# sapeirone/EgoPack

Measured on AMD Instinct MI355X. Metric: clip-seqs/sec training, AR+LTA+PNR multi-task, higher is better.
Workload: dtype bf16; 1 GPU; MTL pre-train AR+LTA+PNR (BASELINE config 3): per GPU B=64 seqs/task x T=32 nodes, 3x1536-d Omnivore-shaped features, H=1024, TRN hidden 1024 (dropout 0.5), depth 3, k=1, Adam; graph mode, fused backbone pass; global_batch=192, parallelism=dp1, trainable_params=25003272, capture=one graph, input=resident in HBM before the timed region, master_weights=f32, mode=bf16, activations=bf16

## Files before the change

__graft_entry__.py:

```python
from __future__ import annotations

import subprocess
import sys
from pathlib import Path

REPO = Path(__file__).resolve().parent
if str(REPO) not in sys.path:
    sys.path.insert(0, str(REPO))


def build() -> None:
    from egopack_amd import build as b
    lib = b.build_library(force=False, verbose=False)
    assert lib.exists()
    from egopack_amd import _lib
    handle = _lib.load()
    missing = [s for s in [*_lib.header_symbols(), *_lib.optim_header_symbols(), *_lib.optim_groups_header_symbols(),
                            *_lib.ema_header_symbols(), *_lib.ce_balanced_header_symbols(),
                            *_lib.bce_balanced_header_symbols()] if not hasattr(handle, s)]
    if missing:
        raise RuntimeError(f"libegopack_hip.so does not export: {missing}")
    import egopack_amd.engine
    import egopack_amd.models


def smoke() -> None:
    import torch
    if not torch.cuda.is_available():
        raise RuntimeError("smoke() needs a GPU")
    build()
    from egopack_amd import data as D
    from egopack_amd import engine, ops
    from egopack_amd.criterion import BCEWithLogitsNone, CrossEntropyNone, MetricSelectorWrapper
    from egopack_amd.models import Graph
    from egopack_amd.models.tasks import LTATask, OSCCTask, PNRTask, RecognitionTask
    from egopack_amd.optim import FlatAdam
    from oracle import path as O
    from oracle import pyg_ops as P

    torch.manual_seed(1)
    F_IN, S, H, HP, heads = 64, 3, 128, 96, (13, 17)
    trn = {"_target_": "egopack_amd.models.temporal_pooling.trn_pooling.TRNPooling", "dropout": 0.0, "hidden_size": HP}
    model = Graph(F_IN, hidden_size=H, depth=3, temporal_pooling=trn, num_segments=S)
    tasks = {"ar": RecognitionTask(H, H, heads), "oscc": OSCCTask(H, H), "lta": LTATask(H, H, heads), "pnr": PNRTask(H, H)}
    names = {"ar": "task/recognition", "oscc": "task/oscc", "lta": "task/lta", "pnr": "task/pnr"}
    sds = {"temporal_graph": {k: v.clone() for k, v in model.state_dict().items()}}
    for t, n in names.items():
        sds[n] = {k: v.clone() for k, v in tasks[t].state_dict().items()}
    host = {}
    for t, T in (("ar", 9), ("lta", 12), ("pnr", 8)):
        ds = D.SyntheticTaskDataset(t, 4, T, S, F_IN, heads, k=1, seed=3)
        host[t] = D.collate([ds[i] for i in range(4)])
    weights = {"ar": 1.0, "oscc": 0.0, "lta": 0.5, "pnr": 2.0}

    class DS:
        has_joint_label, num_labels = False, 2
    crit = {"ar": MetricSelectorWrapper(CrossEntropyNone(), DS()), "lta": MetricSelectorWrapper(CrossEntropyNone(), DS()),
            "oscc": CrossEntropyNone(), "pnr": BCEWithLogitsNone()}
    model.cuda()
    for t in tasks.values():
        t.cuda()
    params = [*model.parameters(), *(p for t in tasks.values() for p in t.parameters())]
    opt = FlatAdam(params, lr=1e-3, weight_decay=1e-5)
    step = engine.MTLStep(model, tasks, crit, weights, opt, fused_backbone=True)
    dev = {t: b.to("cuda") for t, b in host.items()}
    with ops.compute_mode("f32"):
        total, vectors = step.step(dev)
    torch.cuda.synchronize()

    leaf = {g: {k: (v.clone().requires_grad_(True) if v.is_floating_point() and not k.endswith("frequency") else v)
                for k, v in sd.items()} for g, sd in sds.items()}
    obatches = {t: P.OData(**{k: v for k, v in b.__dict__.items() if torch.is_tensor(v) or k == "num_graphs"})
# ... 19 lines not shown
```

egopack_amd/_lib.py:

```python
from __future__ import annotations

import ctypes as C
import os
import re
from pathlib import Path

import torch

HERE = Path(__file__).resolve().parent
LIB_PATH = Path(os.environ["EGK_LIB_PATH"]) if os.environ.get("EGK_LIB_PATH") else HERE / "libegopack_hip.so"
HEADER = HERE.parent / "include" / "egopack_hip.h"
OPTIM_HEADER = HERE.parent / "include" / "egopack_optim.h"
OPTIM_GROUPS_HEADER = HERE.parent / "include" / "egopack_optim_groups.h"

EMA_HEADER = HERE.parent / "include" / "egopack_ema.h"
CE_BALANCED_HEADER = HERE.parent / "include" / "egopack_ce_balanced.h"
BCE_BALANCED_HEADER = HERE.parent / "include" / "egopack_bce_balanced.h"

vp, i32, i64, u64, f32 = C.c_void_p, C.c_int32, C.c_int64, C.c_uint64, C.c_float


class GemmDesc(C.Structure):
    _fields_ = [
        ("M", i32), ("N", i32), ("K1", i32), ("K2", i32),
        ("A1", vp), ("A2", vp), ("B1", vp), ("B2", vp),
        ("lda1", i64), ("lda2", i64), ("ldb1", i64), ("ldb2", i64),
        ("transA", i32), ("transB", i32), ("a_dtype", i32), ("b_dtype", i32),
        ("compute", i32),
        ("C", vp), ("ldc", i64), ("c_dtype", i32),
        ("accumulate", i32), ("act", i32), ("alpha", f32),
        ("bias", vp), ("residual", vp), ("ldr", i64), ("r_dtype", i32),
        ("splitk", i32), ("ws", vp), ("ws_bytes", i64), ("dbias", vp),
        ("st_mode", i32), ("st_nseg", i32), ("st_min_seg_rows", i32), ("st_seg_ptr", vp), ("st_ws", vp), ("st_x", vp),
        ("st_ldx", i64), ("st_stats", vp), ("st_w", vp), ("st_b", vp), ("st_slope", f32),
        ("n_extra", i32), ("xK", i32 * 4), ("xA", vp * 4), ("xB", vp * 4), ("xlda", i64 * 4), ("xldb", i64 * 4),
        ("op_f16", i32),
    ]


class HostDataset(C.Structure):
    _fields_ = [("T", i32), ("S", i32), ("train", i32), ("y_heads", i32), ("L", i64), ("y_elems", i64), ("heavy_in_launch", i64),
                ("live_share", C.c_double),
                ("y", vp), ("pos", vp), ("tau", vp), ("first", vp), ("vlen", vp), ("starts", vp), ("ends", vp),
                ("n_tmpl", i64), ("e_max", i64), ("h_max", i64), ("th_max", i64),
                ("t_e", vp), ("t_ei", vp), ("t_col", vp), ("t_tcol", vp), ("t_tw", vp), ("t_rp", vp), ("t_trp", vp), ("t_band", vp),
                ("t_nh", vp), ("t_nth", vp), ("t_hv", vp), ("t_thv", vp), ("t_dmax", vp), ("t_tdmax", vp)]


class HostBatch(C.Structure):
    _fields_ = [("E", i64), ("heavy_cap", i64), ("t_heavy_cap", i64), ("live_cap", i64),
                ("y", vp), ("pos", vp), ("batch", vp), ("ptr", vp), ("ptr32", vp), ("x_idx", vp), ("edge_index", vp),
                ("rowptr", vp), ("col", vp), ("t_rowptr", vp), ("t_col", vp), ("t_wgt", vp), ("band", vp), ("heavy", vp), ("t_heavy", vp),
                ("live_idx", vp), ("live_inv", vp), ("live_y", vp),
                ("n_heavy", i64), ("n_t_heavy", i64), ("n_live", i64), ("pos_min", i64), ("pos_max", i64),
                ("heavy_mode", i32), ("t_heavy_mode", i32), ("edge_cap", i64), ("live_ap_first", i64), ("live_ap_step", i64)]


class HostPart(C.Structure):
    _fields_ = [("n_nodes", i64), ("E", i64), ("n_heavy", i64), ("n_t_heavy", i64), ("edge_stride", i64), ("pos_min", i64), ("pos_max", i64),
                ("pos", vp), ("edge_index", vp), ("rowptr", vp), ("col", vp), ("t_rowptr", vp), ("t_col", vp), ("t_wgt", vp), ("band", vp),
                ("heavy", vp), ("t_heavy", vp), ("heavy_mode", i32), ("t_heavy_mode", i32)]


class HostMerged(C.Structure):
    _fields_ = [("edge_cap", i64), ("pos", vp), ("edge_index", vp), ("rowptr", vp), ("col", vp), ("t_rowptr", vp), ("t_col", vp),
                ("t_wgt", vp), ("band", vp), ("heavy", vp), ("t_heavy", vp), ("seg_ptr", vp),
                ("n_nodes", i64), ("E", i64), ("min_seg_rows", i64), ("pos_min", i64), ("pos_max", i64),
                ("heavy_mode", i32), ("t_heavy_mode", i32)]


class CETask(C.Structure):
    _fields_ = [("logits", vp * 4), ("ld", i64 * 4), ("C", i32 * 4), ("pad", i32 * 4), ("dcol", i64 * 4), ("n_heads", i32),
                ("y", vp), ("y_stride", i64), ("loss", vp), ("dlogits", vp), ("ldd", i64), ("rows", i32), ("gscale", f32)]


class CEWTask(C.Structure):
    _fields_ = [("base", CETask), ("weight", vp * 4), ("offset", vp * 4)]


class OptimDesc(C.Structure):
    _fields_ = [("rule", i32), ("g_dtype", i32), ("n", i64), ("p", vp), ("g", vp), ("state0", vp), ("state1", vp), ("hyper", vp),
                ("t_dev", vp), ("beta1", C.c_double), ("beta2", C.c_double), ("eps", f32), ("weight_decay", f32), ("momentum", f32), ("dampening", f32),
                ("nesterov", i32), ("bf16_shadow", vp), ("bf16_lo_shadow", vp), ("bump_word", vp), ("bump", i64), ("gate", vp)]


class OptimGroups(C.Structure):
    _fields_ = [("base", i64), ("n_seg", i32), ("n_groups", i32), ("seg_begin", vp), ("seg_group", vp), ("group_hyper", vp)]


class EmaDesc(C.Structure):
    _fields_ = [("ema", vp), ("decay", C.c_double), ("warmup", i32)]


OPT_ADAM, OPT_ADAMW, OPT_SGD = 0, 1, 2

SIGNATURES = {
    "egk_version": (C.c_int, []),
    "egk_last_error": (C.c_char_p, []),
    "egk_prof_enable": (C.c_int, [C.c_int]),
    "egk_prof_reset": (C.c_int, []),
    "egk_prof_count": (C.c_int, []),
    "egk_prof_get": (C.c_int, [C.c_int, C.c_char_p, C.c_int, C.POINTER(i64), C.POINTER(C.c_double),
                               C.POINTER(C.c_double), C.POINTER(C.c_double)]),
    "egk_stamp": (C.c_int, [vp, vp, i32]),
    "egk_tee_split_next": (C.c_int, [vp, vp, i64]),
    "egk_gemm": (C.c_int, [vp, C.POINTER(GemmDesc)]),
    "egk_gemm_stats_blocks": (C.c_int, [C.POINTER(GemmDesc)]),
    "egk_gemm_grouped": (C.c_int, [vp, C.POINTER(GemmDesc), i32]),
    "egk_gemm_ws_bytes": (i64, [C.POINTER(GemmDesc)]),
    "egk_gemm_splitk": (C.c_int, [i32, i32, i32, i32]),
    "egk_gemm_set_pipeline": (C.c_int, [i32]),
    "egk_colsum_ws_len": (C.c_int, [i32, i32]),
    "egk_colsum": (C.c_int, [vp, vp, i64, i32, i32, vp, i32, vp, i32]),
    "egk_rowln_fwd": (C.c_int, [vp, vp, vp, vp, vp, vp, vp, vp, i32, i32, f32, i32, f32, u64, u64, vp, i32]),
    "egk_rowln_bwd_ws_rows": (C.c_int, [i32]),
    "egk_rowln_bwd": (C.c_int, [vp, vp, vp, vp, vp, vp, vp, vp, vp, vp, vp, vp, i32, i32, i32, f32, i32]),
    "egk_ln_bwd_reduce": (C.c_int, [vp, vp, vp, vp, i32, i32, i32]),
    "egk_ln_bwd_reduce_multi": (C.c_int, [vp, vp, vp, vp, vp, vp, vp, i32]),
    "egk_rowln_group_fwd": (C.c_int, [vp, vp, vp, vp, vp, i32, vp, vp, vp, i32, f32, i32, i32]),
    "egk_rowln_group_bwd": (C.c_int, [vp, vp, vp, vp, vp, vp, i32, vp, vp, vp, vp, i32, i32, i32]),
    "egk_graphln_ws_bytes": (i64, [i32, i32, i32]),
    "egk_graphln_fwd": (C.c_int, [vp, vp, vp, vp, vp, vp, vp, i32, i32, i32, f32, f32, vp, i32]),
    "egk_graphln_bwd": (C.c_int, [vp, vp, vp, vp, vp, vp, vp, vp, vp, vp, i32, i32, i32, f32, f32, vp, i32]),
    "egk_rowdot_ws_rows": (i32, [i32]),
    "egk_rowdot_bce": (C.c_int, [vp, vp, vp, vp, vp, vp, vp, vp, vp, i32, i32, f32, i32]),
    "egk_rowdot_reduce": (C.c_int, [vp, vp, vp, vp, i32, i32]),
    "egk_rowdot_ce2_max_rows": (i32, []),
    "egk_rowdot_ce2": (C.c_int, [vp, vp, vp, vp, vp, vp, vp, vp, vp, vp, vp, i32, i32, f32, f32, i32]),
    "egk_rowdot_ce2_multi": (C.c_int, [vp, i32, vp, vp, vp, vp, vp, vp, vp, vp, vp, vp, i32, i32, i32, f32, f32, i32]),
    "egk_graphln_stats_blocks": (i32, [i32]),
    "egk_graphln_stats": (C.c_int, [vp, vp, vp, i32, i32, i32, vp, i32]),
    "egk_graphln_bwd_stats": (C.c_int, [vp, vp, vp, vp, vp, vp, vp, i32, i32, i32, f32, vp, i32]),
    "egk_graphln_bwd_finish": (C.c_int, [vp, vp, vp, vp, vp, vp, vp, vp, vp, vp, i32, i32, i32, f32, f32, vp, i32, vp, i32]),
    "egk_graphln_fwd_apply": (C.c_int, [vp, vp, vp, vp, vp, vp, vp, i32, i32, i32, f32, f32, vp, i32, i32]),
    "egk_graphln_bwd_apply": (C.c_int, [vp, vp, vp, vp, vp, vp, vp, vp, i32, i32, i32, f32, f32, vp, i32, vp, i32]),
    "egk_pe_table": (C.c_int, [vp, vp, i64, i32, i32, vp]),
    "egk_pe_add_table": (C.c_int, [vp, vp, vp, vp, vp, i64, i32, vp, i32, i32, i32]),
    "egk_pe_add": (C.c_int, [vp, vp, vp, vp, vp, i32, i32, i32]),
    "egk_csr_gather": (C.c_int, [vp, vp, vp, vp, vp, vp, vp, i32, i32, i32, vp, i32, vp, i32]),
    "egk_csr_gather_banded": (C.c_int, [vp, vp, vp, vp, vp, vp, i32, i32, i32, vp, i32, vp, i32]),
    "egk_csr_heavy_ws_bytes": (i64, [i32, i32]),
    "egk_csr_heavy_threshold": (i32, []),
    "egk_gather_max_fwd": (C.c_int, [vp, vp, vp, vp, vp, vp, i32, i32, i32, i32]),
    "egk_gather_max_group_fwd": (C.c_int, [vp, vp, vp, vp, i32, vp, vp, i32, i32, i32, i32]),
    "egk_gather_max_tune": (C.c_int, [i32]),
# ... 42 lines not shown
    "egk_weighted_sums_acc": (C.c_int, [vp, vp, vp, vp, i32, vp, vp]),
    "egk_fill_scaled_multi": (C.c_int, [vp, vp, vp, vp, vp, i32]),
    "egk_copy_blocks": (C.c_int, [vp, vp, vp, vp, i32]),
    "egk_gather_rows": (C.c_int, [vp, vp, i32, i64, i64, vp, vp, i32, i64, i32]),
    "egk_gather_lerp_rows": (C.c_int, [vp, vp, i32, i64, i64, vp, vp, vp, vp, i32, i64, i32]),
    "egk_label_rank": (C.c_int, [vp, vp, i64, vp, i64, vp, i32, i32]),
    "egk_edit_distance": (C.c_int, [vp, vp, i64, i64, i64, vp, i64, i64, vp, i32, i32, i32]),
    "egk_cast_rows": (C.c_int, [vp, vp, i32, i64, vp, i32, i64, i32, i32, i32]),
    "egk_axpby": (C.c_int, [vp, vp, vp, vp, i64, f32, f32]),
    "egk_fill_scaled": (C.c_int, [vp, vp, f32, vp, i64]),
    "egk_sum_scale": (C.c_int, [vp, vp, vp, i64, f32, i32]),
    "egk_adam_step": (C.c_int, [vp, vp, vp, i32, vp, vp, i64, vp, f32, f32, f32, f32, vp]),
    "egk_zero_fill": (C.c_int, [vp, vp, i64]),
    "egk_zero_fill_ranges": (C.c_int, [vp, vp, vp, vp, i32]),
    "egk_adam_step_bump": (C.c_int, [vp, vp, vp, i32, vp, vp, i64, vp, f32, f32, f32, f32, vp, vp, vp, i64]),
    "egk_adam_hyper": (C.c_int, [vp, vp, vp, C.c_double, C.c_double, vp]),
    "egk_grad_sumsq_slots": (C.c_int, [i64]),
    "egk_grad_sumsq": (C.c_int, [vp, vp, i32, i64, vp, i32]),
    "egk_grad_norm_finalize": (C.c_int, [vp, vp, i32, vp, f32, vp, vp, vp, vp]),
    "egk_adam_step_gated": (C.c_int, [vp, vp, vp, i32, vp, vp, i64, vp, f32, f32, f32, f32, vp, vp, vp, i64, vp]),
}


OPTIM_SIGNATURES = {
    "egk_optim_step": (C.c_int, [vp, C.POINTER(OptimDesc)]),
}


OPTIM_GROUPS_SIGNATURES = {
    "egk_optim_step_groups": (C.c_int, [vp, C.POINTER(OptimDesc), C.POINTER(OptimGroups)]),
}


EMA_SIGNATURES = {
    "egk_optim_step_ema": (C.c_int, [vp, C.POINTER(OptimDesc), C.POINTER(OptimGroups), C.POINTER(EmaDesc)]),
    "egk_ema_swap": (C.c_int, [vp, vp, vp, i64]),
}


CE_BALANCED_SIGNATURES = {
    "egk_ce_w_fwd": (C.c_int, [vp, vp, i64, vp, i64, vp, vp, vp, vp, i32, i32, f32, i32]),
    "egk_ce_w_bwd": (C.c_int, [vp, vp, i64, vp, i64, vp, vp, vp, vp, vp, i64, i32, i32, f32, i32]),
    "egk_ce_w_fused_multi": (C.c_int, [vp, C.POINTER(CEWTask), i32, f32, i32]),
}


BCE_BALANCED_SIGNATURES = {
    "egk_bce_w_fwd": (C.c_int, [vp, vp, vp, vp, i32, f32, f32, f32]),
    "egk_bce_w_bwd": (C.c_int, [vp, vp, vp, vp, vp, i32, f32, f32, f32, i32]),
    "egk_rowdot_bce_w": (C.c_int, [vp, vp, vp, vp, vp, vp, vp, vp, vp, i32, i32, f32, f32, f32, f32, i32]),
}


def _declared(header: Path) -> list:
    text = header.read_text()
    text = re.sub(r"/\*.*?\*/", "", text, flags=re.S)
    return sorted(set(re.findall(r"\b(egk_[a-z0-9_]+)\s*\(", text)))


def header_symbols() -> list:
    return _declared(HEADER)


def optim_header_symbols() -> list:
    return _declared(OPTIM_HEADER)


def optim_groups_header_symbols() -> list:
    return _declared(OPTIM_GROUPS_HEADER)


def ema_header_symbols() -> list:
    return _declared(EMA_HEADER)


def ce_balanced_header_symbols() -> list:
    return _declared(CE_BALANCED_HEADER)


def bce_balanced_header_symbols() -> list:
    return _declared(BCE_BALANCED_HEADER)


_lib = None


def load() -> C.CDLL:
    global _lib
    if _lib is not None:
        return _lib
    if not LIB_PATH.exists():
        raise RuntimeError(
            f"{LIB_PATH} is missing: build it with `python -m egopack_amd.build` "
            "(or __graft_entry__.build()).  egopack_amd has no CPU / eager fallback.")
    lib = C.CDLL(str(LIB_PATH))
    for name, (res, args) in [*SIGNATURES.items(), *OPTIM_SIGNATURES.items(), *OPTIM_GROUPS_SIGNATURES.items(),
                              *EMA_SIGNATURES.items(), *CE_BALANCED_SIGNATURES.items(), *BCE_BALANCED_SIGNATURES.items()]:
        fn = getattr(lib, name)
        fn.restype = res
        fn.argtypes = args
    _lib = lib
    return lib


def last_error() -> str:
    return load().egk_last_error().decode(errors="replace")
```

egopack_amd/csrc/common.h:

```cpp
#pragma once
#include <hip/hip_runtime.h>
#include <stdint.h>
#include <stdio.h>

#include <initializer_list>

#include "../../include/egopack_hip.h"

namespace egk {

void set_error(const char* fmt, ...);

#define EGK_REQUIRE(cond, ...)               \
    do {                                     \
        if (!(cond)) {                       \
            ::egk::set_error(__VA_ARGS__);   \
            return EGK_EINVAL;               \
        }                                    \
    } while (0)

inline bool aligned_to(unsigned bytes, std::initializer_list<const void*> ps) {
    for (const void* p : ps)
        if (reinterpret_cast<uintptr_t>(p) & (bytes - 1)) return false;
    return true;
// ... 97 lines not shown

struct RowWalk {
    int first, end, step;
};
__device__ __forceinline__ RowWalk row_walk(int blk, int nblk, int row0, int rows, int wave, int wpb) {
    if (nblk >= 8 && (nblk & 7) == 0) {
        const int xcd = blk & 7, slot = blk >> 3, nslot = nblk >> 3;
        const int per = (((rows - row0 + 7) >> 3) + wpb - 1) / wpb * wpb;
        const int b = row0 + xcd * per;
        const int e = b + per < rows ? b + per : rows;
        return RowWalk{b + slot * wpb + wave, e, nslot * wpb};
    }
    return RowWalk{row0 + blk * wpb + wave, rows, nblk * wpb};
}

__device__ __forceinline__ float wave_sum(float v) {
#pragma unroll
    for (int o = 32; o > 0; o >>= 1) v += __shfl_xor(v, o, 64);
    return v;
}
__device__ __forceinline__ double wave_sum(double v) {
#pragma unroll
    for (int o = 32; o > 0; o >>= 1) v += __shfl_xor(v, o, 64);
    return v;
}
__device__ __forceinline__ float wave_max(float v) {
#pragma unroll
    for (int o = 32; o > 0; o >>= 1) v = fmaxf(v, __shfl_xor(v, o, 64));
    return v;
}

__device__ __forceinline__ uint4 philox4x32_10(uint64_t ctr, uint64_t seed) {
    uint32_t c0 = (uint32_t)ctr, c1 = (uint32_t)(ctr >> 32), c2 = 0, c3 = 0;
    uint32_t k0 = (uint32_t)seed, k1 = (uint32_t)(seed >> 32);
#pragma unroll
    for (int r = 0; r < 10; ++r) {
        uint32_t hi0 = __umulhi(0xD2511F53u, c0), lo0 = 0xD2511F53u * c0;
        uint32_t hi1 = __umulhi(0xCD9E8D57u, c2), lo1 = 0xCD9E8D57u * c2;
        uint32_t n0 = hi1 ^ c1 ^ k0, n1 = lo1, n2 = hi0 ^ c3 ^ k1, n3 = lo0;
        c0 = n0; c1 = n1; c2 = n2; c3 = n3;
        k0 += 0x9E3779B9u; k1 += 0xBB67AE85u;
    }
    return make_uint4(c0, c1, c2, c3);
}
__device__ __forceinline__ float u01(uint32_t r) { return (float)(r >> 8) * (1.0f / 16777216.0f); }

inline int cdiv(int64_t a, int64_t b) { return (int)((a + b - 1) / b); }

typedef unsigned short bf16_t;

__device__ __forceinline__ float bf2f(bf16_t h) { return __uint_as_float((unsigned)h << 16); }
__device__ __forceinline__ bf16_t f2bf(float f) { return __builtin_bit_cast(bf16_t, (__bf16)f); }

__device__ __forceinline__ float4 ld4t(const float* __restrict__ p, int c, int cols, bool vec) {
    if (vec && c + 4 <= cols) return *reinterpret_cast<const float4*>(p + c);
    float4 v;
    v.x = c + 0 < cols ? p[c + 0] : 0.f;
    v.y = c + 1 < cols ? p[c + 1] : 0.f;
    v.z = c + 2 < cols ? p[c + 2] : 0.f;
    v.w = c + 3 < cols ? p[c + 3] : 0.f;
    return v;
}
__device__ __forceinline__ float4 ld4t(const bf16_t* __restrict__ p, int c, int cols, bool vec) {
    float4 v;
    if (vec && c + 4 <= cols) {
        const uint2 r = *reinterpret_cast<const uint2*>(p + c);
        v.x = __uint_as_float(r.x << 16); v.y = __uint_as_float(r.x & 0xffff0000u);
        v.z = __uint_as_float(r.y << 16); v.w = __uint_as_float(r.y & 0xffff0000u);
        return v;
    }
    v.x = c + 0 < cols ? bf2f(p[c + 0]) : 0.f;
    v.y = c + 1 < cols ? bf2f(p[c + 1]) : 0.f;
    v.z = c + 2 < cols ? bf2f(p[c + 2]) : 0.f;
    v.w = c + 3 < cols ? bf2f(p[c + 3]) : 0.f;
    return v;
}
__device__ __forceinline__ void st4t(float* __restrict__ p, int c, int cols, bool vec, float4 v) {
    if (vec && c + 4 <= cols) {
        *reinterpret_cast<float4*>(p + c) = v;
        return;
    }
    if (c + 0 < cols) p[c + 0] = v.x;
    if (c + 1 < cols) p[c + 1] = v.y;
    if (c + 2 < cols) p[c + 2] = v.z;
    if (c + 3 < cols) p[c + 3] = v.w;
}
__device__ __forceinline__ void st4t(bf16_t* __restrict__ p, int c, int cols, bool vec, float4 v) {
    if (vec && c + 4 <= cols) {
        uint2 pk;
        pk.x = (unsigned)f2bf(v.x) | ((unsigned)f2bf(v.y) << 16);
        pk.y = (unsigned)f2bf(v.z) | ((unsigned)f2bf(v.w) << 16);
        *reinterpret_cast<uint2*>(p + c) = pk;
        return;
    }
    if (c + 0 < cols) p[c + 0] = f2bf(v.x);
    if (c + 1 < cols) p[c + 1] = f2bf(v.y);
    if (c + 2 < cols) p[c + 2] = f2bf(v.z);
    if (c + 3 < cols) p[c + 3] = f2bf(v.w);
}
__device__ __forceinline__ float ld1t(const float* p) { return *p; }
__device__ __forceinline__ float ld1t(const bf16_t* p) { return bf2f(*p); }
__device__ __forceinline__ void st1t(float* p, float v) { *p = v; }
__device__ __forceinline__ void st1t(bf16_t* p, float v) { *p = f2bf(v); }

struct SplitTee {
    bf16_t* hi;
// ... 59 lines not shown
```

egopack_amd/csrc/gemm.hip:

```cpp
#include <type_traits>

#include "common.h"

namespace egk {

typedef __attribute__((ext_vector_type(4))) float f32x4;
typedef __attribute__((ext_vector_type(8))) __bf16 bf16x8;
typedef unsigned short bf16_t;

constexpr int BM = 128, BN = 128, ROWB = 128;
constexpr int NTHREADS = 256;

constexpr int MAXSRC = 6;
struct GemmArgs {
    int M, N;
    int nsrc;
    int K[MAXSRC];
    const void* A[MAXSRC];
    const void* B[MAXSRC];
    long long lda[MAXSRC], ldb[MAXSRC];
    int a_vec, b_vec;
    void* C;
    long long ldc;
    int c_vec, c_bf16;
// ... 416 lines not shown
            if (g.c_bf16) {
                const uint4 r = *reinterpret_cast<const uint4*>((const bf16_t*)g.st_x + (long long)m * g.st_ldx + n);
                const unsigned rw[4] = {r.x, r.y, r.z, r.w};
#pragma unroll
                for (int t = 0; t < 4; ++t) {
                    xv[2 * t] = __uint_as_float(rw[t] << 16);
                    xv[2 * t + 1] = __uint_as_float(rw[t] & 0xffff0000u);
                }
            } else {
                const float* xp = (const float*)g.st_x + (long long)m * g.st_ldx + n;
                const float4 x0 = *reinterpret_cast<const float4*>(xp), x1 = *reinterpret_cast<const float4*>(xp + 4);
                xv[0] = x0.x; xv[1] = x0.y; xv[2] = x0.z; xv[3] = x0.w; xv[4] = x1.x; xv[5] = x1.y; xv[6] = x1.z; xv[7] = x1.w;
            }
            float a1 = 0.f, a2 = 0.f;
#pragma unroll
            for (int t = 0; t < 8; ++t) {
                const float xh = (xv[t] - mu) * ri;
                const float pre = xh * lw[t] + lb[t];
                const float dxh = o[t] * (pre > 0.f ? 1.f : g.st_slope) * lw[t];
                a1 += dxh;
                a2 += dxh * xh;
            }
            sa[rel][0] += a1;
            sa[rel][1] += a2;
        }
    }
    if constexpr (ST) if (st_mode) {
        __shared__ double st_red_static[MBW == 1 ? 4 : 1][4];
        double (*st_red)[4] = st_red_static;
        if constexpr (MBW == 2) st_red = reinterpret_cast<double (*)[4]>(lds + 32 * NI * MBW * 512);
        double v4[4] = {(double)sa[0][0], (double)sa[0][1], (double)sa[1][0], (double)sa[1][1]};
#pragma unroll
        for (int q = 0; q < 4; ++q)
#pragma unroll
            for (int o_ = 32; o_ > 0; o_ >>= 1) v4[q] += __shfl_xor(v4[q], o_, 64);
        if ((tid & 63) == 0) {
#pragma unroll
            for (int q = 0; q < 4; ++q) st_red[tid >> 6][q] = v4[q];
        }
        __syncthreads();
        if (tid < g.st_nseg * 2) {
            const int sg = tid >> 1, k = tid & 1, rel = sg - s0;
            double t_ = 0.0;
            if (rel == 0 || rel == 1) {
                t_ = (st_red[0][rel * 2 + k] + st_red[1][rel * 2 + k]) + (st_red[2][rel * 2 + k] + st_red[3][rel * 2 + k]);
                if constexpr (MBW == 2)
                    t_ += (st_red[4][rel * 2 + k] + st_red[5][rel * 2 + k]) + (st_red[6][rel * 2 + k] + st_red[7][rel * 2 + k]);
            }
            g.st_ws[((long long)st_tile * g.st_nseg + sg) * 2 + k] = t_;
        }
    }
}

template <bool BF16C, bool TA, bool TB, typename AT, typename BT>
__global__ __launch_bounds__(NTHREADS) void gemm_kernel(const GemmArgs g) {
    __shared__ __attribute__((aligned(16))) unsigned char lds[2 * BM * ROWB];
    unsigned char* ldsA = lds;
    unsigned char* ldsB = lds + BM * ROWB;
    constexpr int KT = BF16C ? 64 : 32;
    constexpr bool A16 = sizeof(AT) == 2, B16 = sizeof(BT) == 2;

    const int nwg = g.tiles_m * g.tiles_n;
    int bid = blockIdx.x;
    {
        const int xcd = bid & 7, q = nwg >> 3, r = nwg & 7;
        bid = (xcd < r ? xcd * (q + 1) : r * (q + 1) + (xcd - r) * q) + (bid >> 3);
    }
    const int tm = bid / g.tiles_n, tn = bid % g.tiles_n;
    const int m0 = tm * BM, n0 = tn * BN;

    const int nkt = total_tiles(g, KT);
    const int z = blockIdx.y;
    const int per = (nkt + g.splitk - 1) / g.splitk;
    const int t_begin = z * per, t_end = min(nkt, t_begin + per);

    const int tid = threadIdx.x, lane = tid & 63, w = tid >> 6;
    const int wm = w >> 1, wn = w & 1;
    const int lr = lane & 15, lg = lane >> 4;

    f32x4 acc[4][4];
#pragma unroll
    for (int i = 0; i < 4; ++i)
#pragma unroll
        for (int j = 0; j < 4; ++j) acc[i][j] = f32x4{0.f, 0.f, 0.f, 0.f};

    uint4 ra[8], rb[8];
    auto load_tile = [&](int t) {
        int src, tt;
        source_of<KT>(g, t, src, tt);
        const int k0 = tt * KT;
        load_operand<BF16C, TA, AT>(g.A[src], g.lda[src], g.M, m0, k0, g.K[src], (g.a_vec >> src) & 1, 0, ra);
        load_operand<BF16C, TB, BT>(g.B[src], g.ldb[src], g.N, n0, k0, g.K[src], (g.b_vec >> src) & 1, 1, rb);
    };

    if (t_begin < t_end) load_tile(t_begin);
    for (int t = t_begin; t < t_end; ++t) {
        __syncthreads();
        store_lds<TA, A16>(ldsA, ra, 0);
        store_lds<TB, B16>(ldsB, rb, 1);
        __syncthreads();
        if (t + 1 < t_end) load_tile(t + 1);
#pragma unroll
        for (int s = 0; s < 2; ++s) {
            uint4 a[4], b[4];
#pragma unroll
            for (int i = 0; i < 4; ++i)
// ... 31 lines not shown
}

typedef __attribute__((address_space(3))) void lds_void_t;
typedef const __attribute__((address_space(1))) void glb_void_t;

template <bool TR, int NP, int OFF = 0, int TOT = NP>
__device__ __forceinline__ void cursor_init(const bf16_t* (&pp)[TOT], long long& step, const bf16_t* __restrict__ base, long long ld,
                                            int rows_total, int row0, int k0, int first, int lane, int tiles_per_step) {
    const bf16_t** p = pp + OFF;
#pragma unroll
    for (int i = 0; i < NP; ++i) {
        const int piece = (first + i) & 15, sub_row0 = row0 + ((first + i) >> 4) * 128;
        if constexpr (TR) {
            const int k = piece * 4 + (lane >> 4);
            const int c = (lane & 15) ^ (2 * (k & 3) + 8 * ((k >> 3) & 1));
            int col = sub_row0 + c * 8;
            if (col + 8 > ld) col = 0;
            p[i] = base + (long long)(k0 + k) * ld + col;
        } else {
            const int r = piece * 8 + (lane >> 3);
            const int c = (lane & 7) ^ ((r >> 1) & 7);
            p[i] = base + (long long)min(sub_row0 + r, rows_total - 1) * ld + k0 + c * 8;
        }
    }
    step = (TR ? 64 * ld : 64) * tiles_per_step;
}
template <int NP, int OFF = 0, int TOT = NP>
__device__ __forceinline__ void cursor_issue(const bf16_t* (&pp)[TOT], long long step, unsigned char* img, int first) {
    const bf16_t** p = pp + OFF;
#pragma unroll
    for (int i = 0; i < NP; ++i) {
        __builtin_amdgcn_global_load_lds((glb_void_t*)p[i], (lds_void_t*)(img + (first + i) * 1024), 16, 0, 0);
        p[i] += step;
    }
}
template <bool TR, int NP>
struct OperandCursor {
    const bf16_t* p[NP];
    long long step;
    __device__ __forceinline__ void init(const bf16_t* __restrict__ base, long long ld, int rows_total, int row0, int k0,
                                         int first, int lane, int tiles_per_step) {
        cursor_init<TR, NP, 0, NP>(p, step, base, ld, rows_total, row0, k0, first, lane, tiles_per_step);
    }
    __device__ __forceinline__ void issue(unsigned char* img, int first) { cursor_issue<NP, 0, NP>(p, step, img, first); }
};

typedef _Float16 f16x8 __attribute__((ext_vector_type(8)));
template <bool F16>
__device__ __forceinline__ f32x4 mfma16(const uint4& b, const uint4& a, const f32x4& c) {
    if constexpr (F16) return __builtin_amdgcn_mfma_f32_16x16x32_f16(__builtin_bit_cast(f16x8, b), __builtin_bit_cast(f16x8, a), c, 0, 0, 0);
    else return __builtin_amdgcn_mfma_f32_16x16x32_bf16(__builtin_bit_cast(bf16x8, b), __builtin_bit_cast(bf16x8, a), c, 0, 0, 0);
}

template <int NSTAGE, bool TRA, bool TRB, int KG, int MB, int NI = 4, bool VIRT = false, bool F16 = false, int LW = 0>
__device__ __forceinline__ void gemm_pipe_body(const GemmArgs& g, const int bid) {
    static_assert(KG == 1 || MB == 1, "wave groups and the tall tile are alternatives");
    static_assert(NI == 4 || ((NI == 3 || NI == 2) && !TRA && ((MB == 1 && (KG == 1 || NI == 2)) || (MB == 2 && KG == 1 && NI == 3))),
                  "96- / 64-row tiles: row-major A; two wave groups with 64-row tiles only; the tall 8-wave tile with NI = 3");
    constexpr int IMG = 16384, IMG_A = NI == 4 ? MB * IMG : MB * NI * 4096, STAGE = IMG_A + IMG;
    constexpr int NPB = 4 / MB;
    constexpr int LOADS = NI + NPB;
    constexpr int WG = 4 * MB;
    extern __shared__ __attribute__((aligned(16))) unsigned char lds[];
    constexpr int KT = 64;
#ifdef EGK_GEMM_STAMPS
    const unsigned long long ps_entry = __builtin_amdgcn_s_memtime(), ps_rentry = __builtin_amdgcn_s_memrealtime();
    unsigned long long ps_first = 0;
#endif

    int z, tm, tn;
    if constexpr (VIRT) tile_of_virtual(g, bid, z, tm, tn);
    else tile_of(g, bid, z, tm, tn);
    const int m0 = tm * (32 * NI * MB), n0 = tn * BN;
    const int nkt = total_tiles(g, KT);
    const int per = (nkt + g.splitk - 1) / g.splitk;
    const int t_begin = z * per, t_end = min(nkt, t_begin + per);

    const int tid = threadIdx.x, lane = tid & 63;
    const int wall = __builtin_amdgcn_readfirstlane(tid >> 6);
    const int grp = KG == 1 ? 0 : (wall / WG);
    const int w = wall % WG;
    const int wm = w >> 1, wn = w & 1;
    const int lr = lane & 15, lg = lane >> 4;
    unsigned char* ring = lds + grp * (NSTAGE * STAGE);

    const int nt_all = t_end - t_begin;
    const int nt = nt_all > grp ? (nt_all - grp + KG - 1) / KG : 0;
    const int rounds = (nt_all + KG - 1) / KG;

    OperandCursor<TRA, NI> ca;
    OperandCursor<TRB, NPB> cb;
    int cur_src = -1;
    auto issue = [&](int i, int stage) {
        const int t = t_begin + grp + KG * i;
        int src, tt;
        source_of<KT>(g, t, src, tt);
        if (src != cur_src) {
            const int k0 = tt * KT;
            ca.init((const bf16_t*)g.A[src], g.lda[src], g.M, m0, k0, w * NI, lane, KG);
            cb.init((const bf16_t*)g.B[src], g.ldb[src], g.N, n0, k0, w * NPB, lane, KG);
            cur_src = src;
        }
        unsigned char* sbase = ring + stage * STAGE;
        ca.issue(sbase, w * NI);
        cb.issue(sbase + IMG_A, w * NPB);
    };

    if constexpr (LW > 0) {
// ... 147 lines not shown
            for (int j = 0; j < 4; ++j)
                asm volatile("ds_read_b128 %0, %1 offset:%2" : "=v"(b1[j]) : "v"((stB + b_rm) ^ 64u), "n"(j * 2048));
        }
        constexpr int R1 = ((TRA ? 8 : NI) + (TRB ? 8 : 4)) > 15 ? 15 : ((TRA ? 8 : NI) + (TRB ? 8 : 4));
        asm volatile("s_waitcnt lgkmcnt(%0)" ::"n"(R1) : "memory");
        __builtin_amdgcn_sched_barrier(0);
#pragma unroll
        for (int i = 0; i < NI; ++i)
#pragma unroll
            for (int j = 0; j < 4; ++j)
                acc[i][j] = mfma16<F16>(b0[j], a0[i], acc[i][j]);
        asm volatile("s_waitcnt lgkmcnt(0)" ::: "memory");
        __builtin_amdgcn_sched_barrier(0);
#pragma unroll
        for (int i = 0; i < NI; ++i)
#pragma unroll
            for (int j = 0; j < 4; ++j)
                acc[i][j] = mfma16<F16>(b1[j], a1[i], acc[i][j]);
        if constexpr (TRA) {
            if (do_bias) {
#pragma unroll
                for (int r = 0; r < 4; ++r) {
                    const unsigned wv[4] = {bz[r].x, bz[r].y, bz[r].z, bz[r].w};
#pragma unroll
                    for (int e = 0; e < 4; ++e) {
                        bsum[2 * e] += __uint_as_float(wv[e] << 16);
                        bsum[2 * e + 1] += __uint_as_float(wv[e] & 0xffff0000u);
                    }
                }
            }
        }
    }
#ifdef EGK_GEMM_STAMPS
    const unsigned long long ps_loop = __builtin_amdgcn_s_memtime();
#endif
    if constexpr (TRA) {
        if (g.dbias != nullptr && tn == 0) {
            __syncthreads();
            float* red = reinterpret_cast<float*>(lds);
            const int slot = MB == 2 ? bsub : grp;
#pragma unroll
            for (int e = 0; e < 8; ++e) red[(slot * 16 + bkg) * 128 + bcc * 8 + e] = bsum[e];
            __syncthreads();
            if (tid < 128 * MB && m0 + tid < g.M) {
                const int q0 = MB == 2 ? (tid >> 7) * 16 : 0, nq = MB == 2 ? 16 : 16 * KG;
                float t = 0.f;
                for (int q = 0; q < nq; ++q) t += red[(q0 + q) * 128 + (tid & 127)];
                if (g.splitk > 1) g.ws_bias[(long long)z * g.M + m0 + tid] = t;
                else g.dbias[m0 + tid] += t;
            }
            __syncthreads();
        }
    }
    if constexpr (KG == 1) {
        if constexpr (MB == 1) {
            if (epilogue_rows_ok(g)) gemm_epilogue_rows<NI>(g, acc, lds, m0, n0, wm, wn, lr, lg, z, tid, tm * g.tiles_n + tn);
            else gemm_epilogue<NI, 4>(g, acc, m0, n0, wm * 16 * NI, wn * 64, lr, lg, z);
        } else if constexpr (NI == 3) {
            static_assert(NSTAGE * STAGE >= 192 * 512 + 256, "the rows epilogue stages the whole tile (+ the wave partials) in the ring");
            if (epilogue_rows_ok(g)) gemm_epilogue_rows<NI, true, 2>(g, acc, lds, m0, n0, wm, wn, lr, lg, z, tid, tm * g.tiles_n + tn);
            else gemm_epilogue<NI, 4>(g, acc, m0, n0, wm * 16 * NI, wn * 64, lr, lg, z);
        } else {
            gemm_epilogue<NI, 4>(g, acc, m0, n0, wm * 16 * NI, wn * 64, lr, lg, z);
        }
    } else if constexpr (NI == 4 || NI == 2) {
        constexpr int HF = NI / 2;
        __syncthreads();
        f32x4* xch = reinterpret_cast<f32x4*>(lds);
        f32x4* mine_out = xch + ((grp * 4 + w) * (HF * 4)) * 64 + lane;
        const f32x4* theirs = xch + (((1 - grp) * 4 + w) * (HF * 4)) * 64 + lane;
        f32x4 half[HF][4];
        if (grp == 0) {
#pragma unroll
            for (int i = 0; i < HF; ++i)
#pragma unroll
                for (int j = 0; j < 4; ++j) mine_out[(i * 4 + j) * 64] = acc[HF + i][j];
        } else {
#pragma unroll
            for (int i = 0; i < HF; ++i)
#pragma unroll
                for (int j = 0; j < 4; ++j) mine_out[(i * 4 + j) * 64] = acc[i][j];
        }
        __syncthreads();
        if (grp == 0) {
#pragma unroll
            for (int i = 0; i < HF; ++i)
#pragma unroll
                for (int j = 0; j < 4; ++j) half[i][j] = acc[i][j] + theirs[(i * 4 + j) * 64];
        } else {
#pragma unroll
            for (int i = 0; i < HF; ++i)
#pragma unroll
                for (int j = 0; j < 4; ++j) half[i][j] = theirs[(i * 4 + j) * 64] + acc[HF + i][j];
        }
        gemm_epilogue<HF, 4>(g, half, m0, n0, wm * 16 * NI + grp * 16 * HF, wn * 64, lr, lg, z);
    }
#ifdef EGK_GEMM_STAMPS
    if (g.ws_bias != nullptr && g.dbias == nullptr && tid == 0) {
        const unsigned long long ps_issued = __builtin_amdgcn_s_memtime();
        asm volatile("s_waitcnt vmcnt(0)" ::: "memory");
        unsigned long long* o = reinterpret_cast<unsigned long long*>(g.ws_bias) + (long long)bid * 8;
        const unsigned long long ps_end = __builtin_amdgcn_s_memtime();
        o[7] = ps_issued - ps_loop;
        o[0] = ps_first - ps_entry; o[1] = ps_loop - ps_first; o[2] = ps_end - ps_loop; o[3] = ps_end - ps_entry;
        o[4] = __builtin_amdgcn_s_memrealtime() - ps_rentry; o[5] = ps_rentry; o[6] = nt;
    }
#endif
}

__device__ __forceinline__ void splitk_finish_group(const GemmArgs& g, int m, int n, long long total) {
    const long long idx = (long long)m * g.N + n;
    float4 s4 = make_float4(0.f, 0.f, 0.f, 0.f);
    for (int z = 0; z < g.splitk; ++z) {
        const float4 v = *reinterpret_cast<const float4*>(g.ws + (long long)z * total + idx);
        s4.x += v.x; s4.y += v.y; s4.z += v.z; s4.w += v.w;
    }
    float o[4] = {s4.x * g.alpha, s4.y * g.alpha, s4.z * g.alpha, s4.w * g.alpha};
    if (g.accumulate) {
        const float4 c = *reinterpret_cast<const float4*>((const float*)g.C + (long long)m * g.ldc + n);
        o[0] += c.x; o[1] += c.y; o[2] += c.z; o[3] += c.w;
    }
    if (g.bias) {
#pragma unroll
        for (int t = 0; t < 4; ++t) o[t] += g.bias[n + t];
    }
    if (g.act == EGK_ACT_RELU) {
#pragma unroll
        for (int t = 0; t < 4; ++t) o[t] = fmaxf(o[t], 0.f);
    }
    if (g.residual) {
        if (g.r_bf16) {
            const uint2 r = *reinterpret_cast<const uint2*>((const bf16_t*)g.residual + (long long)m * g.ldr + n);
            o[0] += __uint_as_float(r.x << 16); o[1] += __uint_as_float(r.x & 0xffff0000u);
            o[2] += __uint_as_float(r.y << 16); o[3] += __uint_as_float(r.y & 0xffff0000u);
        } else {
            const float4 r = *reinterpret_cast<const float4*>((const float*)g.residual + (long long)m * g.ldr + n);
            o[0] += r.x; o[1] += r.y; o[2] += r.z; o[3] += r.w;
        }
    }
    if (g.c_bf16) {
        uint2 pk;
        pk.x = (unsigned)f32_to_bf16(o[0]) | ((unsigned)f32_to_bf16(o[1]) << 16);
        pk.y = (unsigned)f32_to_bf16(o[2]) | ((unsigned)f32_to_bf16(o[3]) << 16);
        *reinterpret_cast<uint2*>((bf16_t*)g.C + (long long)m * g.ldc + n) = pk;
    } else {
        *reinterpret_cast<float4*>((float*)g.C + (long long)m * g.ldc + n) = make_float4(o[0], o[1], o[2], o[3]);
    }
}

template <int NSTAGE, bool TRA, bool TRB, int KG, int MB, int NI = 4, bool F16 = false, int LW = 0>
__global__ __launch_bounds__(NTHREADS * KG * MB + 64 * LW) void gemm_pipe_kernel(const GemmArgs g) {
    gemm_pipe_body<NSTAGE, TRA, TRB, KG, MB, NI, false, F16, LW>(g, blockIdx.x);
}

constexpr int MAX_GROUPS = 8;
struct GemmGroup {
    GemmArgs p[MAX_GROUPS];
    int packed, count, total;
};
template <int NSTAGE, bool TRA, bool TRB, int KG, int MB, int NI = 4, bool F16 = false, int LW = 0>
__global__ __launch_bounds__(NTHREADS * KG * MB + 64 * LW) void gemm_pipe_group_kernel(const GemmGroup gg) {
    if (gg.packed) {
        const int lin = blockIdx.x, xcd = lin & 7, slot = lin >> 3;
        const int q = gg.total >> 3, r = gg.total & 7;
        if (slot >= q + (xcd < r ? 1 : 0)) return;
        int v = (xcd < r ? xcd * (q + 1) : r * (q + 1) + (xcd - r) * q) + slot;
        int pi = 0;
        for (; pi + 1 < gg.count; ++pi) {
            const int t = gg.p[pi].tiles_m * gg.p[pi].tiles_n;
            if (v < t) break;
            v -= t;
        }
        gemm_pipe_body<NSTAGE, TRA, TRB, KG, MB, NI, true, F16, LW>(gg.p[pi], v);
        return;
    }
    const GemmArgs& g = gg.p[blockIdx.y];
    if ((int)blockIdx.x >= g.tiles_m * g.tiles_n * g.splitk) return;
    gemm_pipe_body<NSTAGE, TRA, TRB, KG, MB, NI, false, F16, LW>(g, blockIdx.x);
}


template <bool TR, int FIRST, int S, int CNT = 4>
__device__ __forceinline__ void read_frags4(uint4 (&dst)[4], unsigned st, unsigned rm, const unsigned* tr) {
    if constexpr (TR) {
#pragma unroll
        for (int i = 0; i < CNT; ++i) {
            const unsigned ad = st + tr[FIRST + i];
            uint2 lo, hi;
            asm volatile("ds_read_b64_tr_b16 %0, %1 offset:%2" : "=v"(lo) : "v"(ad), "n"(S * 8192));
            asm volatile("ds_read_b64_tr_b16 %0, %1 offset:%2" : "=v"(hi) : "v"(ad), "n"(S * 8192 + 1024));
            dst[i] = make_uint4(lo.x, lo.y, hi.x, hi.y);
        }
    } else {
        const unsigned ad = S ? ((st + rm) ^ 64u) : (st + rm);
#pragma unroll
        for (int i = 0; i < CNT; ++i) asm volatile("ds_read_b128 %0, %1 offset:%2" : "=v"(dst[i]) : "v"(ad), "n"((FIRST + i) * 2048));
    }
}
template <int NI, int CNT = 4>
__device__ __forceinline__ void mfma_4x4(f32x4 (&acc)[NI][4], int i0, const uint4 (&a)[4], const uint4 (&b)[4]) {
#pragma unroll
    for (int i = 0; i < CNT; ++i)
#pragma unroll
        for (int j = 0; j < 4; ++j)
            acc[i0 + i][j] = __builtin_amdgcn_mfma_f32_16x16x32_bf16(__builtin_bit_cast(bf16x8, b[j]), __builtin_bit_cast(bf16x8, a[i]),
// ... 400 lines not shown
static int g_use_pipe = 1;
static constexpr double REDUCE_FIXED_US = 3.5;
static int g_r192_loaders = 1;
static int g_tt_tall = 1;
static bool g_lds_attr_set = false;
template <int NS, bool TA, bool TB, int KG, int MB = 1>
static void set_lds_attr() {
    (void)hipFuncSetAttribute((const void*)egk::gemm_pipe_kernel<NS, TA, TB, KG, MB>, hipFuncAttributeMaxDynamicSharedMemorySize,
                              NS * KG * (MB + 1) * 16384);
}
static void ensure_lds_attr() {
    if (g_lds_attr_set) return;
    set_lds_attr<2, false, false, 1>(); set_lds_attr<2, false, true, 1>(); set_lds_attr<2, true, true, 1>(); set_lds_attr<2, true, false, 1>();
    set_lds_attr<2, false, false, 2>(); set_lds_attr<2, false, true, 2>(); set_lds_attr<2, true, true, 2>(); set_lds_attr<2, true, false, 2>();
    (void)hipFuncSetAttribute((const void*)egk::gemm_pipe_kernel<2, false, false, 1, 1, 2>, hipFuncAttributeMaxDynamicSharedMemorySize, 65536);
    (void)hipFuncSetAttribute((const void*)egk::gemm_pipe_kernel<2, false, true, 1, 1, 2>, hipFuncAttributeMaxDynamicSharedMemorySize, 65536);
    (void)hipFuncSetAttribute((const void*)egk::gemm_pipe_kernel<2, false, false, 1, 1, 3>, hipFuncAttributeMaxDynamicSharedMemorySize, 65536);
    (void)hipFuncSetAttribute((const void*)egk::gemm_pipe_kernel<2, false, true, 1, 1, 3>, hipFuncAttributeMaxDynamicSharedMemorySize, 65536);
    (void)hipFuncSetAttribute((const void*)egk::gemm_big_kernel<false, false>, hipFuncAttributeMaxDynamicSharedMemorySize, 131072);
    (void)hipFuncSetAttribute((const void*)egk::gemm_big_kernel<false, true>, hipFuncAttributeMaxDynamicSharedMemorySize, 131072);
    (void)hipFuncSetAttribute((const void*)egk::gemm_big_kernel<true, true>, hipFuncAttributeMaxDynamicSharedMemorySize, 131072);
    (void)hipFuncSetAttribute((const void*)egk::gemm_big_kernel<true, false>, hipFuncAttributeMaxDynamicSharedMemorySize, 131072);
    (void)hipFuncSetAttribute((const void*)egk::gemm_big_kernel<false, false, 8, 6>, hipFuncAttributeMaxDynamicSharedMemorySize, 131072);
    (void)hipFuncSetAttribute((const void*)egk::gemm_big_kernel<false, true, 8, 6>, hipFuncAttributeMaxDynamicSharedMemorySize, 131072);
    (void)hipFuncSetAttribute((const void*)egk::gemm_pipe_group_kernel<2, false, false, 1, 1, 2>, hipFuncAttributeMaxDynamicSharedMemorySize, 65536);
    (void)hipFuncSetAttribute((const void*)egk::gemm_pipe_group_kernel<2, false, true, 1, 1, 2>, hipFuncAttributeMaxDynamicSharedMemorySize, 65536);
    (void)hipFuncSetAttribute((const void*)egk::gemm_pipe_group_kernel<2, false, false, 1, 1, 3>, hipFuncAttributeMaxDynamicSharedMemorySize, 65536);
    (void)hipFuncSetAttribute((const void*)egk::gemm_pipe_group_kernel<2, false, true, 1, 1, 3>, hipFuncAttributeMaxDynamicSharedMemorySize, 65536);
    (void)hipFuncSetAttribute((const void*)egk::gemm_pipe_group_kernel<2, false, false, 1, 1>, hipFuncAttributeMaxDynamicSharedMemorySize, 65536);
    (void)hipFuncSetAttribute((const void*)egk::gemm_pipe_group_kernel<2, false, false, 1, 1, 4, true>, hipFuncAttributeMaxDynamicSharedMemorySize, 65536);
    (void)hipFuncSetAttribute((const void*)egk::gemm_pipe_group_kernel<2, false, true, 1, 1>, hipFuncAttributeMaxDynamicSharedMemorySize, 65536);
    (void)hipFuncSetAttribute((const void*)egk::gemm_pipe_group_kernel<2, true, true, 1, 1>, hipFuncAttributeMaxDynamicSharedMemorySize, 131072);
    (void)hipFuncSetAttribute((const void*)egk::gemm_pipe_group_kernel<2, true, true, 2, 1>, hipFuncAttributeMaxDynamicSharedMemorySize, 131072);
    (void)hipFuncSetAttribute((const void*)egk::gemm_pipe_group_kernel<3, true, true, 1, 2>, hipFuncAttributeMaxDynamicSharedMemorySize, 3 * 49152);
    (void)hipFuncSetAttribute((const void*)egk::gemm_pipe_group_kernel<3, false, false, 1, 2, 3, false, 4>, hipFuncAttributeMaxDynamicSharedMemorySize, 3 * 40960);
    (void)hipFuncSetAttribute((const void*)egk::gemm_pipe_group_kernel<3, false, true, 1, 2, 3, false, 4>, hipFuncAttributeMaxDynamicSharedMemorySize, 3 * 40960);
    (void)hipFuncSetAttribute((const void*)egk::gemm_pipe_group_kernel<2, false, false, 2, 1>, hipFuncAttributeMaxDynamicSharedMemorySize, 131072);
    (void)hipFuncSetAttribute((const void*)egk::gemm_pipe_group_kernel<2, false, true, 2, 1>, hipFuncAttributeMaxDynamicSharedMemorySize, 131072);
    (void)hipFuncSetAttribute((const void*)egk::gemm_pipe_f32_kernel<false, false>, hipFuncAttributeMaxDynamicSharedMemorySize, 65536);
    (void)hipFuncSetAttribute((const void*)egk::gemm_pipe_f32_kernel<false, true>, hipFuncAttributeMaxDynamicSharedMemorySize, 65536);
    (void)hipFuncSetAttribute((const void*)egk::gemm_pipe_f32_kernel<true, true>, hipFuncAttributeMaxDynamicSharedMemorySize, 65536);
    (void)hipFuncSetAttribute((const void*)egk::gemm_pipe_f32_kernel<true, false>, hipFuncAttributeMaxDynamicSharedMemorySize, 65536);
    (void)hipFuncSetAttribute((const void*)egk::gemm_pipe_f32_group_kernel<false, false>, hipFuncAttributeMaxDynamicSharedMemorySize, 65536);
    (void)hipFuncSetAttribute((const void*)egk::gemm_pipe_f32_group_kernel<false, true>, hipFuncAttributeMaxDynamicSharedMemorySize, 65536);
    (void)hipFuncSetAttribute((const void*)egk::gemm_pipe_f32_group_kernel<true, true>, hipFuncAttributeMaxDynamicSharedMemorySize, 65536);
    (void)hipFuncSetAttribute((const void*)egk::gemm_pipe_f32_kernel<false, false, 3>, hipFuncAttributeMaxDynamicSharedMemorySize, 65536);
    (void)hipFuncSetAttribute((const void*)egk::gemm_pipe_f32_kernel<false, true, 3>, hipFuncAttributeMaxDynamicSharedMemorySize, 65536);
    (void)hipFuncSetAttribute((const void*)egk::gemm_pipe_kernel<3, false, false, 1, 2, 3>, hipFuncAttributeMaxDynamicSharedMemorySize, 3 * 40960);
    (void)hipFuncSetAttribute((const void*)egk::gemm_pipe_kernel<3, false, true, 1, 2, 3>, hipFuncAttributeMaxDynamicSharedMemorySize, 3 * 40960);
    (void)hipFuncSetAttribute((const void*)egk::gemm_pipe_kernel<3, false, false, 1, 2, 3, false, 4>, hipFuncAttributeMaxDynamicSharedMemorySize, 3 * 40960);
    (void)hipFuncSetAttribute((const void*)egk::gemm_pipe_kernel<3, false, true, 1, 2, 3, false, 4>, hipFuncAttributeMaxDynamicSharedMemorySize, 3 * 40960);
    (void)hipFuncSetAttribute((const void*)egk::gemm_pipe_kernel<2, false, false, 2, 1, 2>, hipFuncAttributeMaxDynamicSharedMemorySize, 4 * 24576);
    (void)hipFuncSetAttribute((const void*)egk::gemm_pipe_kernel<2, false, true, 2, 1, 2>, hipFuncAttributeMaxDynamicSharedMemorySize, 4 * 24576);
    g_lds_attr_set = true;
}
extern "C" int egk_gemm_set_pipeline(int32_t on) {
    const int prev = g_use_pipe;
    if (on == 870 || on == 871) { g_r192_loaders = on - 870; return prev; }
    if (on == 850 || on == 851) { g_tt_tall = on - 850; return prev; }
    if (on < 0 || on >= 20) return -1;
    g_use_pipe = on;
    return prev;
}

extern "C" int egk_gemm_splitk(int32_t M, int32_t N, int32_t K, int32_t compute) {
    const int KT = compute == EGK_COMPUTE_BF16 ? 64 : 32;
    const int tiles = cdiv(M, BM) * cdiv(N, BN);
    const int nkt = cdiv(K, KT);
    if (compute != EGK_COMPUTE_BF16) {
        if (nkt < 8) return 1;
        const double mn = (double)M * N / 1048576.0;
        const long long t96 = (long long)cdiv(M, 96) * cdiv(N, BN);
        auto rounds = [&](int s_) {
            const double r128 = (double)cdiv((long long)tiles * s_, 256), r96 = 0.75 * cdiv(t96 * s_, 256);
            return r128 < r96 ? r128 : r96;
        };
        int best = 1;
        double best_cost = rounds(1) * nkt * 1.9;
        for (int s = 2; s <= 16 && nkt / s >= 4; ++s) {
            const double cost = rounds(s) * cdiv(nkt, s) * 1.9 + 3.5 + 1.5 * s * mn;
            if (cost < 0.93 * best_cost) { best_cost = cost; best = s; }
        }
        return best;
    }
    if (tiles > 128 || nkt < 4) return 1;
    const double mn = (double)M * N / 1048576.0;
    int best = 1;
    double best_cost = 6.5 + 0.45 * nkt;
    for (int s = 2; s <= 16 && tiles * s <= 256 && nkt / s >= 2; s *= 2) {
        const double cost = 6.5 + 0.45 * cdiv(nkt, s) + REDUCE_FIXED_US + 1.5 * s * mn;
        if (cost < best_cost - 0.5) { best_cost = cost; best = s; }
    }
    return best;
}

extern "C" int64_t egk_gemm_ws_bytes(const egk_gemm_desc* d) {
    if (!d) return 0;
    const int sk = d->splitk > 1 ? d->splitk : 1;
    int64_t n = sk > 1 ? (int64_t)sk * d->M * d->N * 4 : 0;
    if (d->dbias) {
        const int64_t fused = sk > 1 ? (int64_t)sk * d->M * 4 : 0;
        const int64_t plain = (int64_t)egk_colsum_ws_len(d->K1, d->M) * 4;
        n += fused > plain ? fused : plain;
    }
    return n;
}

struct SourceInfo {
    long long k_total = 0;
    bool all_k64 = true, all_vec = true;
};
static int fill_sources(const egk_gemm_desc* d, GemmArgs& g, int ea, int eb, SourceInfo& info, const char* who) {
    EGK_REQUIRE(d->n_extra >= 0 && d->n_extra <= MAXSRC - 2, "%s: n_extra must be 0 .. %d", who, MAXSRC - 2);
    g.nsrc = 0;
    g.a_vec = g.b_vec = 0;
    for (int i = 0; i < MAXSRC; ++i) { g.K[i] = 0; g.A[i] = g.B[i] = nullptr; g.lda[i] = g.ldb[i] = 0; }
    auto add = [&](const void* A, const void* B, long long lda, long long ldb, int K) -> int {
        EGK_REQUIRE(K >= 0, "%s: negative K", who);
        if (K == 0) return 0;
        EGK_REQUIRE(A && B, "%s: null operand of a non-empty K source", who);
        const int i = g.nsrc++;
        g.K[i] = K; g.A[i] = A; g.B[i] = B; g.lda[i] = lda; g.ldb[i] = ldb;
        const bool av = aligned16(A) && (lda % ea == 0), bv = aligned16(B) && (ldb % eb == 0);
        g.a_vec |= (av ? 1 : 0) << i;
        g.b_vec |= (bv ? 1 : 0) << i;
        info.k_total += K;
        info.all_k64 = info.all_k64 && (K % 64 == 0);
        info.all_vec = info.all_vec && av && bv;
        return 0;
    };
    int rc = add(d->A1, d->B1, d->lda1, d->ldb1, d->K1);
    if (rc) return rc;
    rc = add(d->A2, d->B2, d->lda2, d->ldb2, d->K2);
    if (rc) return rc;
    for (int i = 0; i < d->n_extra; ++i) {
        rc = add(d->xA[i], d->xB[i], d->xlda[i], d->xldb[i], d->xK[i]);
        if (rc) return rc;
    }
    if (g.nsrc == 0) g.nsrc = 1;
    return 0;
}

static int gemm_core(egk_stream_t stream, const egk_gemm_desc* d, int* query_blocks);

extern "C" int egk_gemm(egk_stream_t stream, const egk_gemm_desc* d) { return gemm_core(stream, d, nullptr); }

extern "C" int egk_gemm_stats_blocks(const egk_gemm_desc* d) {
    int blocks = 0;
    const int rc = gemm_core(nullptr, d, &blocks);
    return rc == 0 ? blocks : 0;
}

static int gemm_core(egk_stream_t stream, const egk_gemm_desc* d, int* query_blocks) {
    EGK_REQUIRE(d != nullptr, "egk_gemm: null descriptor");
    EGK_REQUIRE(d->M >= 0 && d->N >= 0 && d->K1 >= 0 && d->K2 >= 0, "egk_gemm: negative size");
    EGK_REQUIRE(d->compute == EGK_COMPUTE_F32 || d->compute == EGK_COMPUTE_BF16, "egk_gemm: bad compute type");
    EGK_REQUIRE(!d->op_f16, "egk_gemm: op_f16 is a grouped-launch feature (egk_gemm_grouped with >= 2 problems)");
    const bool a16 = d->a_dtype == EGK_BF16, b16 = d->b_dtype == EGK_BF16;
    EGK_REQUIRE((d->a_dtype == EGK_F32 || a16) && (d->b_dtype == EGK_F32 || b16) &&
                    (d->c_dtype == EGK_F32 || d->c_dtype == EGK_BF16) &&
                    (d->r_dtype == EGK_F32 || d->r_dtype == EGK_BF16),
                "egk_gemm: unknown element type");
    EGK_REQUIRE(a16 == b16, "egk_gemm: A and B must have the same element type in memory");
    EGK_REQUIRE(!(a16 && d->compute == EGK_COMPUTE_F32), "egk_gemm: bf16 operands need EGK_COMPUTE_BF16");
    EGK_REQUIRE(!(d->accumulate && d->c_dtype != EGK_F32), "egk_gemm: accumulate needs an f32 C");
    EGK_REQUIRE(d->C != nullptr || d->M == 0 || d->N == 0, "egk_gemm: null C");
    if (d->M == 0 || d->N == 0) return 0;
    hipStream_t s = (hipStream_t)stream;

    GemmArgs g;
    g.M = d->M; g.N = d->N;
    const int ea = a16 ? 8 : 4, eb = b16 ? 8 : 4;
    SourceInfo src;
    {
        const int rc = fill_sources(d, g, ea, eb, src, "egk_gemm");
        if (rc) return rc;
    }
    g.C = d->C; g.ldc = d->ldc;
    g.c_bf16 = d->c_dtype == EGK_BF16;
    g.c_vec = g.c_bf16 ? ((reinterpret_cast<uintptr_t>(g.C) & 7) == 0 && g.ldc % 4 == 0) : (aligned16(g.C) && g.ldc % 4 == 0);
    g.accumulate = d->accumulate; g.act = d->act; g.alpha = d->alpha;
    g.bias = d->bias; g.residual = d->residual; g.ldr = d->ldr;
    g.r_bf16 = d->r_dtype == EGK_BF16;
    g.r_vec = g.residual && (g.r_bf16 ? ((reinterpret_cast<uintptr_t>(g.residual) & 7) == 0 && g.ldr % 4 == 0)
                                      : (aligned16(g.residual) && g.ldr % 4 == 0));
    g.splitk = d->splitk > 1 ? d->splitk : 1;
    g.ws = (float*)d->ws;
    if (g.splitk > 1)
        EGK_REQUIRE(g.ws && d->ws_bytes >= (int64_t)g.splitk * d->M * d->N * 4, "egk_gemm: split-K workspace too small");
    g.tiles_m = cdiv(g.M, BM); g.tiles_n = cdiv(g.N, BN);
    g.dbias = nullptr; g.ws_bias = nullptr;
    g.group_m = 1;
    g.rows_epilogue = 1;
    g.st_mode = d->st_mode; g.st_nseg = d->st_nseg; g.st_seg_ptr = d->st_seg_ptr; g.st_ws = (double*)d->st_ws;
    g.st_x = d->st_x; g.st_ldx = d->st_ldx; g.st_stats = d->st_stats; g.st_w = d->st_w; g.st_b = d->st_b; g.st_slope = d->st_slope;
    if (d->st_mode) {
        EGK_REQUIRE(d->st_mode == 1 || d->st_mode == 2, "egk_gemm: st_mode must be 0, 1 or 2");
        EGK_REQUIRE(d->st_nseg >= 1 && d->st_nseg <= 16 && d->st_seg_ptr && (query_blocks || d->st_ws), "egk_gemm: st_* segments / workspace");
        EGK_REQUIRE(d->st_mode == 1 || (d->st_x && d->st_stats && d->st_w && d->st_b), "egk_gemm: st_mode 2 needs x, stats, w, b");
    }
    if (query_blocks) *query_blocks = 0;
    const long long K = src.k_total;
    const double flops = 2.0 * d->M * d->N * K;
    const double bytes = (a16 ? 2.0 : 4.0) * ((double)d->M * K + (double)d->N * K) + (g.c_bf16 ? 2.0 : 4.0) * d->M * d->N;
    const int bf = d->compute == EGK_COMPUTE_BF16;
    const int layout = d->transA ? (d->transB ? 2 : 3) : (d->transB ? 1 : 0);
    const double slab_bytes = d->splitk > 1 ? ((double)d->splitk + 1.0) * d->M * d->N * 4.0 : 0.0;

    const bool pipe_ok = bf && a16 && g_use_pipe && src.all_k64 && K > 0 && src.all_vec;
    const bool single = d->K2 == 0 && d->n_extra == 0;
    bool all_k32 = K > 0;
    for (int i = 0; i < g.nsrc; ++i) all_k32 = all_k32 && (g.K[i] % 32 == 0);
    const bool pipe32_ok = !bf && !a16 && g_use_pipe && all_k32 && src.all_vec;
    const bool bias_fused = (pipe_ok || pipe32_ok) && d->dbias && d->transA && single;
    if (d->dbias) {
        EGK_REQUIRE(d->transA && single, "egk_gemm: dbias needs the dW form (transA, single K source)");
        const int64_t slab = g.splitk > 1 ? (int64_t)g.splitk * d->M * d->N * 4 : 0;
        const int64_t need = bias_fused ? slab + (g.splitk > 1 ? (int64_t)g.splitk * d->M * 4 : 0)
                                        : slab + (int64_t)egk_colsum_ws_len(d->K1, d->M) * 4;
        EGK_REQUIRE(d->ws && d->ws_bytes >= need, "egk_gemm: workspace too small for dbias (%lld bytes needed)", (long long)need);
        if (bias_fused) {
            g.dbias = d->dbias;
            g.ws_bias = g.splitk > 1 ? (float*)((char*)d->ws + slab) : nullptr;
        } else if (!query_blocks) {
            const int rc = egk_colsum(stream, d->A1, d->lda1, d->K1, d->M, d->dbias, 1, (float*)((char*)d->ws + slab), d->a_dtype);
            if (rc) return rc;
        }
    }
    if (pipe_ok) {
        ensure_lds_attr();
        dim3 pblock(NTHREADS);
        const int nwg128 = g.tiles_m * g.tiles_n * g.splitk;
        const int nkt_slab = cdiv(K / 64, g.splitk);
        int variant = g_use_pipe;
        if (variant == 1) {
            variant = nwg128 > 256 ? 3 : (nkt_slab >= 4 ? 5 : 3);
            if (!d->transA && g.splitk == 1) {
                const long long t128 = (long long)cdiv(g.M, 128) * g.tiles_n, t96 = (long long)cdiv(g.M, 96) * g.tiles_n;
                const long long t64 = (long long)cdiv(g.M, 64) * g.tiles_n;
                if (nwg128 > 256) {
                    if (((t96 + 255) / 256) * 28 < ((t128 + 255) / 256) * 32) variant = 8;
                    const long long t192 = (long long)cdiv(g.M, 192) * g.tiles_n;
                    const long long cur = variant == 8 ? ((t96 + 255) / 256) * 28 : ((t128 + 255) / 256) * 32;
                    if (t192 > 192 && t192 <= 256 && 40 < cur) variant = 16;
                } else if (t64 <= 256 && t64 > t128) {
                    variant = 11;
                }
            }
            const long long t256 = (long long)cdiv(g.M, 256) * cdiv(g.N, 256);
            if (g.splitk == 1 && !g.dbias && g.M % 256 == 0 && g.N % 256 == 0 && t256 >= 192 && K >= 3072 &&
                10 * t256 >= 9 * 256 * ((t256 + 255) / 256))
                variant = 7;
            const long long t192 = (long long)cdiv(g.M, 192) * cdiv(g.N, 256);
            if (variant != 7 && !d->transA && g.splitk == 1 && !g.dbias && g.M % 192 == 0 && g.N % 256 == 0 && t192 >= 192 && K >= 1024 &&
                10 * t192 >= 9 * 256 * ((t192 + 255) / 256))
                variant = 15;
        } else if ((variant == 8 || variant == 11 || variant == 12 || variant == 16) &&
                   (d->transA || (variant == 16 && g.splitk > 1))) {
            variant = 3;
        } else if (variant == 7 && (g.dbias || g.M % 256 != 0 || g.N % 256 != 0)) {
            variant = 3;
        } else if (variant == 15 && (d->transA || g.dbias || g.M % 192 != 0 || g.N % 256 != 0)) {
            variant = 3;
        }
        if (variant != 3 && variant != 5 && variant != 7 && variant != 8 && variant != 11 && variant != 12 && variant != 15 && variant != 16)
            variant = 3;
        if (variant == 12 && d->st_mode) variant = 11;
        g.tiles_m = variant == 8 ? cdiv(g.M, 96) : (variant == 11 || variant == 12) ? cdiv(g.M, 64) : variant == 7 ? cdiv(g.M, 256)
                    : (variant == 15 || variant == 16) ? cdiv(g.M, 192) : cdiv(g.M, BM);
        if (variant == 7 || variant == 15) g.tiles_n = cdiv(g.N, 256);
#ifdef EGK_GEMM_STAMPS
        if (variant != 7 && !g.dbias && d->ws) {
            const int64_t slab = g.splitk > 1 ? (int64_t)g.splitk * d->M * d->N * 4 : 0;
            if (d->ws_bytes >= slab + (int64_t)g.tiles_m * g.tiles_n * g.splitk * 64) g.ws_bias = (float*)((char*)d->ws + slab);
        }
        if (variant == 7 && g.splitk == 1 && !g.dbias && d->ws && d->ws_bytes >= (int64_t)g.tiles_m * g.tiles_n * 8 * 64)
            g.ws_bias = (float*)d->ws;
#endif
        {
            const int tiles = g.tiles_m * g.tiles_n;
            int per_xcd = cdiv(tiles * g.splitk, 8);
            if (per_xcd > tiles) per_xcd = tiles;
            int gm = 1;
            while ((gm + 1) * (gm + 1) <= per_xcd) ++gm;
            g.group_m = gm < g.tiles_m ? gm : g.tiles_m;
            if (!d->transA && g.splitk == 1 && g.tiles_m % 8 == 0) g.group_m = g.tiles_m / 8;
        }

        const int tile_rows = variant == 8 ? 96 : (variant == 11 || variant == 12) ? 64 : variant == 16 ? 192 : 128;
        const bool st_ok = (variant == 3 || variant == 8 || variant == 11 || variant == 16) && g.splitk == 1 &&
                           epilogue_rows_ok(g) && d->st_min_seg_rows >= tile_rows &&
                           (d->st_mode != 2 || (aligned16(d->st_x) && d->st_ldx % (g.c_bf16 ? 8 : 4) == 0 && aligned16(d->st_w) && aligned16(d->st_b)));
        if (query_blocks) {
            *query_blocks = (d->st_mode && st_ok) ? g.tiles_m * g.tiles_n : 0;
            return 0;
        }
        if (d->st_mode && !st_ok) {
            set_error("egk_gemm: st_mode %d is not available for this launch (ask egk_gemm_stats_blocks first)", d->st_mode);
            return EGK_EUNSUPPORTED;
        }
        dim3 pgrid(g.tiles_m * g.tiles_n * g.splitk);
#define EGK_PIPE(TA, TB)                                                                                                  \
    do {                                                                                                                  \
        if (variant == 16 && g_r192_loaders && nkt_slab >= 4) {                                                           \
            hipLaunchKernelGGL((gemm_pipe_kernel<3, false, TB, 1, 2, 3, false, 4>), pgrid, dim3(2 * NTHREADS + 256), 3 * 40960, s, g); \
        } else if (variant == 16) {                                                                                       \
            hipLaunchKernelGGL((gemm_pipe_kernel<3, false, TB, 1, 2, 3>), pgrid, dim3(2 * NTHREADS), 3 * 40960, s, g);    \
        } else if (variant == 15) {                                                                                       \
            hipLaunchKernelGGL((gemm_big_kernel<false, TB, 8, 6>), pgrid, dim3(512), 131072, s, g);                       \
        } else if (variant == 7) {                                                                                        \
            hipLaunchKernelGGL((gemm_big_kernel<TA, TB>), pgrid, dim3(512), 131072, s, g);                                \
        } else if (variant == 12) {                                                                                       \
            hipLaunchKernelGGL((gemm_pipe_kernel<2, false, TB, 2, 1, 2>), pgrid, dim3(2 * NTHREADS), 4 * 24576, s, g);    \
        } else if (variant == 11) {                                                                                       \
            hipLaunchKernelGGL((gemm_pipe_kernel<2, false, TB, 1, 1, 2>), pgrid, pblock, 2 * 24576, s, g);                \
        } else if (variant == 8) {                                                                                        \
            hipLaunchKernelGGL((gemm_pipe_kernel<2, false, TB, 1, 1, 3>), pgrid, pblock, 2 * 28672, s, g);                \
        } else if (variant == 5)                                                                                          \
            hipLaunchKernelGGL((gemm_pipe_kernel<2, TA, TB, 2, 1>), pgrid, dim3(2 * NTHREADS), 4 * 32768, s, g);          \
        else hipLaunchKernelGGL((gemm_pipe_kernel<2, TA, TB, 1, 1>), pgrid, pblock, 2 * 32768, s, g);                     \
    } while (0)
        {
            ProfScope prof((variant == 7 || variant == 15) ? KID_GEMM_BF16_NN_T256 + layout : variant == 8 ? KID_GEMM_BF16_NN_R96 + layout : variant == 11 ? KID_GEMM_BF16_NN_R64 + layout
                                       : variant == 16 ? KID_GEMM_BF16_NN_R192 + layout
                                       : ((variant == 5 || variant == 12) ? KID_GEMM_BF16_NN_G2 : KID_GEMM_BF16_NN) + layout, s, flops, bytes);
            if (!d->transA && !d->transB) EGK_PIPE(false, false);
            else if (!d->transA && d->transB) EGK_PIPE(false, true);
            else if (d->transA && d->transB) EGK_PIPE(true, true);
            else EGK_PIPE(true, false);
        }
#undef EGK_PIPE
        const bool defer = take_defer_reduce();
        if (defer)
            EGK_REQUIRE(g.splitk > 1 && !g.accumulate && g.act == 0 && !g.residual && g.alpha == 1.f && !g.c_bf16 && !g.dbias,
                        "egk_gemm_defer_reduce_next: a split launch with a plain f32 result (bias only)");
        if (g.splitk > 1 && !defer) {
            ProfScope prof(KID_GEMM_SPLITK_REDUCE, s, 0, slab_bytes);
            const long long total = (long long)g.M * g.N;
            const long long work = (total + 3) / 4;
            hipLaunchKernelGGL(gemm_splitk_reduce, dim3((unsigned)((work + 255) / 256 < 2048 ? (work + 255) / 256 : 2048)),
                               dim3(256), 0, s, g);
        }
        return check_launch("egk_gemm");
    }
    if (pipe32_ok) {
        ensure_lds_attr();
        bool r96 = false;
        if (!d->transA && g_use_pipe != 3) {
            const long long t128 = (long long)cdiv(g.M, 128) * g.tiles_n * g.splitk, t96 = (long long)cdiv(g.M, 96) * g.tiles_n * g.splitk;
            r96 = g_use_pipe == 8 || ((t96 + 255) / 256) * 96 < ((t128 + 255) / 256) * 128;
        }
        if (r96) g.tiles_m = cdiv(g.M, 96);
        {
            const int tiles = g.tiles_m * g.tiles_n;
            int per_xcd = cdiv(tiles * g.splitk, 8);
            if (per_xcd > tiles) per_xcd = tiles;
            int gm = 1;
            while ((gm + 1) * (gm + 1) <= per_xcd) ++gm;
            g.group_m = gm < g.tiles_m ? gm : g.tiles_m;
            if (!d->transA && g.splitk == 1 && g.tiles_m % 8 == 0) g.group_m = g.tiles_m / 8;
        }
        const bool st_ok = g.splitk == 1 && epilogue_rows_ok(g) && d->st_min_seg_rows >= (r96 ? 96 : 128) &&
                           (d->st_mode != 2 || (aligned16(d->st_x) && d->st_ldx % 4 == 0 && aligned16(d->st_w) && aligned16(d->st_b)));
        if (query_blocks) {
            *query_blocks = (d->st_mode && st_ok) ? g.tiles_m * g.tiles_n : 0;
            return 0;
        }
        if (d->st_mode && !st_ok) {
            set_error("egk_gemm: st_mode %d is not available for this launch (ask egk_gemm_stats_blocks first)", d->st_mode);
            return EGK_EUNSUPPORTED;
        }
        const dim3 pgrid(g.tiles_m * g.tiles_n * g.splitk), pblock(NTHREADS);
        {
            ProfScope prof(KID_GEMM_F32_NN + layout, s, flops, bytes);
            if (r96 && !d->transB) hipLaunchKernelGGL((gemm_pipe_f32_kernel<false, false, 3>), pgrid, pblock, 2 * 28672, s, g);
            else if (r96) hipLaunchKernelGGL((gemm_pipe_f32_kernel<false, true, 3>), pgrid, pblock, 2 * 28672, s, g);
            else if (!d->transA && !d->transB) hipLaunchKernelGGL((gemm_pipe_f32_kernel<false, false>), pgrid, pblock, 65536, s, g);
            else if (!d->transA && d->transB) hipLaunchKernelGGL((gemm_pipe_f32_kernel<false, true>), pgrid, pblock, 65536, s, g);
            else if (d->transA && d->transB) hipLaunchKernelGGL((gemm_pipe_f32_kernel<true, true>), pgrid, pblock, 65536, s, g);
            else hipLaunchKernelGGL((gemm_pipe_f32_kernel<true, false>), pgrid, pblock, 65536, s, g);
        }
        EGK_REQUIRE(!take_defer_reduce(), "egk_gemm_defer_reduce_next: only the bf16-operand pipelined launches leave their slabs");
        if (g.splitk > 1) {
            ProfScope prof(KID_GEMM_SPLITK_REDUCE, s, 0, slab_bytes);
            const long long total = (long long)g.M * g.N;
            const long long work = (total + 3) / 4;
            hipLaunchKernelGGL(gemm_splitk_reduce, dim3((unsigned)((work + 255) / 256 < 2048 ? (work + 255) / 256 : 2048)),
                               dim3(256), 0, s, g);
        }
        return check_launch("egk_gemm");
    }
    if (query_blocks) return 0;
    if (d->st_mode) {
        set_error("egk_gemm: st_mode %d is not available on the generic kernel (ask egk_gemm_stats_blocks first)", d->st_mode);
        return EGK_EUNSUPPORTED;
    }
// ... 197 lines not shown
```

egopack_amd/csrc/graph_ops.hip:

```cpp
#include <math.h>

#include "common.h"
#include "rows1024.h"

namespace egk {

constexpr int WPB = 4;

#define ld4 ld4t
#define st4 st4t

template <typename T>
__global__ __launch_bounds__(256) void pe_add_kernel(const T* __restrict__ x, const long long* __restrict__ pos,
                                                     const float* __restrict__ freq, T* __restrict__ y, int rows,
                                                     int cols, const SplitTee tee) {
    const int lane = threadIdx.x & 63, wave = threadIdx.x >> 6;
    const bool vec = (cols & 3) == 0;
    const int half = cols >> 1;
    const RowWalk rw = row_walk(blockIdx.x, gridDim.x, 0, rows, wave, WPB);
    for (int row = rw.first; row < rw.end; row += rw.step) {
        const float p = (float)pos[row];
        const T* xr = x + (long long)row * cols;
        T* yr = y + (long long)row * cols;
        for (int c = lane * 4; c < cols; c += 256) {
// ... 310 lines not shown
                    }
                cnt = __popc(code[k] & 7u);
            } else {
                const int e0 = rowptr[row], e1 = rowptr[row + 1];
                cnt = e1 - e0;
                if (cnt > skip_above) continue;
                for (int e = e0; e < e1; e += 4) {
                    r1k::Raw t[4];
#pragma unroll
                    for (int u = 0; u < 4; ++u)
                        if (e + u < e1) t[u] = r1k::ld_raw(x + (long long)col[e + u] * r1k::COLS, lane);
#pragma unroll
                    for (int u = 0; u < 4; ++u)
                        if (e + u < e1) {
                            float v[16];
                            r1k::unpack(t[u], v);
#pragma unroll
                            for (int j = 0; j < 16; ++j) acc[j] += 1.f * v[j];
                        }
                }
            }
            const float mean_w = cnt ? 1.f / (float)cnt : 0.f;
#pragma unroll
            for (int j = 0; j < 16; ++j) acc[j] *= mean_w;
            r1k::st_raw(out + (long long)row * r1k::COLS, lane, r1k::pack(acc));
            __builtin_amdgcn_sched_barrier(0);
        }
    }
}

template <bool WGT, bool GATE>
__global__ __launch_bounds__(256, 5) void csr_gather_1k_kernel(const bf16_t* __restrict__ x, const int* __restrict__ rowptr,
                                                               const int* __restrict__ col, const float* __restrict__ wgt,
                                                               const bf16_t* __restrict__ gate, bf16_t* __restrict__ out, int rows,
                                                               int skip_above, const int* __restrict__ block_rows, int n_block_rows) {
    const int lane = threadIdx.x & 63, wave = __builtin_amdgcn_readfirstlane(threadIdx.x >> 6);
    if ((int)blockIdx.x < n_block_rows) {
        const int row = block_rows[blockIdx.x];
        const int e0 = rowptr[row], e1 = rowptr[row + 1];
        const long long c = (long long)wave * 256 + lane * 4;
        float a0 = 0.f, a1 = 0.f, a2 = 0.f, a3 = 0.f;
        for (int e = e0; e < e1; e += 8) {
            uint2 v[8];
            float w[8];
#pragma unroll
            for (int u = 0; u < 8; ++u)
                if (e + u < e1) {
                    v[u] = *reinterpret_cast<const uint2*>(x + (long long)col[e + u] * r1k::COLS + c);
                    w[u] = WGT ? wgt[e + u] : 1.f;
                }
#pragma unroll
            for (int u = 0; u < 8; ++u)
                if (e + u < e1) {
                    a0 += w[u] * __uint_as_float(v[u].x << 16); a1 += w[u] * __uint_as_float(v[u].x & 0xffff0000u);
                    a2 += w[u] * __uint_as_float(v[u].y << 16); a3 += w[u] * __uint_as_float(v[u].y & 0xffff0000u);
                }
        }
        if (!WGT) {
            const float mw = e1 > e0 ? 1.f / (float)(e1 - e0) : 0.f;
            a0 *= mw; a1 *= mw; a2 *= mw; a3 *= mw;
        }
        if (GATE) {
            const uint2 gq = *reinterpret_cast<const uint2*>(gate + (long long)row * r1k::COLS + c);
            a0 = __uint_as_float(gq.x << 16) > 0.f ? a0 : 0.f; a1 = __uint_as_float(gq.x & 0xffff0000u) > 0.f ? a1 : 0.f;
            a2 = __uint_as_float(gq.y << 16) > 0.f ? a2 : 0.f; a3 = __uint_as_float(gq.y & 0xffff0000u) > 0.f ? a3 : 0.f;
        }
        uint2 o;
        o.x = (unsigned)f2bf(a0) | ((unsigned)f2bf(a1) << 16);
        o.y = (unsigned)f2bf(a2) | ((unsigned)f2bf(a3) << 16);
        *reinterpret_cast<uint2*>(out + (long long)row * r1k::COLS + c) = o;
        return;
    }
    const int bid = blockIdx.x - n_block_rows, nblk = gridDim.x - n_block_rows;
    const RowWalk rw = (n_block_rows & 7) == 0 ? row_walk(bid, nblk, 0, rows, wave, WPB) : RowWalk{bid * WPB + wave, rows, nblk * WPB};
    for (int row = rw.first; row < rw.end; row += rw.step) {
        const int e0 = rowptr[row], e1 = rowptr[row + 1];
        if (e1 - e0 > skip_above) continue;
        r1k::Raw gt;
        if (GATE) gt = r1k::ld_raw(gate + (long long)row * r1k::COLS, lane);
        float acc[16];
#pragma unroll
        for (int j = 0; j < 16; ++j) acc[j] = 0.f;
        for (int e = e0; e < e1; e += 4) {
            r1k::Raw t[4];
            float w[4];
#pragma unroll
            for (int u = 0; u < 4; ++u)
                if (e + u < e1) {
                    t[u] = r1k::ld_raw(x + (long long)col[e + u] * r1k::COLS, lane);
                    w[u] = WGT ? wgt[e + u] : 1.f;
                }
#pragma unroll
            for (int u = 0; u < 4; ++u)
                if (e + u < e1) {
                    float v[16];
                    r1k::unpack(t[u], v);
#pragma unroll
                    for (int j = 0; j < 16; ++j) acc[j] += w[u] * v[j];
                }
        }
        if (!WGT) {
            const float mw = e1 > e0 ? 1.f / (float)(e1 - e0) : 0.f;
#pragma unroll
            for (int j = 0; j < 16; ++j) acc[j] *= mw;
        }
        if (GATE) {
            float gv[16];
            r1k::unpack(gt, gv);
#pragma unroll
            for (int j = 0; j < 16; ++j) acc[j] = gv[j] > 0.f ? acc[j] : 0.f;
        }
        r1k::st_raw(out + (long long)row * r1k::COLS, lane, r1k::pack(acc));
    }
}

template <int RB>
__global__ __launch_bounds__(256) void pe_add_table_1k_kernel(const bf16_t* __restrict__ x, const long long* __restrict__ pos,
                                                              const float* __restrict__ freq, const float* __restrict__ table,
                                                              long long pos_min, int n_pos, bf16_t* __restrict__ y, int rows) {
    const int lane = threadIdx.x & 63, wave = threadIdx.x >> 6;
    const RowWalk rw = row_walk(blockIdx.x, gridDim.x, 0, rows, wave, WPB);
    const int W = rw.step, rend = rw.end;
    for (int base = rw.first; base < rend; base += RB * W) {
        r1k::Raw raw[RB];
        long long pr[RB];
#pragma unroll
        for (int k = 0; k < RB; ++k)
            if (base + k * W < rend) {
                raw[k] = r1k::ld_raw(x + (long long)(base + k * W) * r1k::COLS, lane);
                pr[k] = pos[base + k * W];
            }
#pragma unroll
        for (int k = 0; k < RB; ++k) {
            const int row = base + k * W;
            if (row >= rend) break;
            const long long ti = pr[k] - pos_min;
            const bool hit = ti >= 0 && ti < n_pos;
            float v[16], e[16];
            r1k::unpack(raw[k], v);
            if (hit) {
                r1k::ld_vec16(table + ti * r1k::COLS, lane, e);
            } else {
#pragma unroll
                for (int j = 0; j < 16; ++j) {
                    const int cc = r1k::col_of(lane, j);
                    const bool is_sin = cc < 512;
                    const float a = (float)pr[k] * freq[is_sin ? cc : cc - 512];
                    e[j] = is_sin ? sinf(a) : cosf(a);
                }
            }
#pragma unroll
            for (int j = 0; j < 16; ++j) v[j] += e[j];
            r1k::st_raw(y + (long long)row * r1k::COLS, lane, r1k::pack(v));
            __builtin_amdgcn_sched_barrier(0);
        }
    }
}

constexpr int VERY_HEAVY = 24, CSR_CHUNKS = 8;

template <typename T>
__global__ __launch_bounds__(256) void csr_heavy_partial_kernel(const T* __restrict__ x, const int* __restrict__ rowptr,
                                                                const int* __restrict__ col, const float* __restrict__ wgt,
// ... 1469 lines not shown
```

egopack_amd/csrc/rows1024.h:

```cpp
#pragma once
#include "common.h"

namespace egk {
namespace r1k {

constexpr int COLS = 1024;

struct Raw {
    uint4 c0, c1;
};

__device__ __forceinline__ Raw ld_raw(const bf16_t* __restrict__ row, int lane) {
    Raw r;
    r.c0 = *reinterpret_cast<const uint4*>(row + 8 * lane);
    r.c1 = *reinterpret_cast<const uint4*>(row + 512 + 8 * lane);
    return r;
}
__device__ __forceinline__ void st_raw(bf16_t* __restrict__ row, int lane, const Raw& r) {
    *reinterpret_cast<uint4*>(row + 8 * lane) = r.c0;
    *reinterpret_cast<uint4*>(row + 512 + 8 * lane) = r.c1;
}
__device__ __forceinline__ void unpack(const Raw& r, float (&f)[16]) {
    const unsigned w[8] = {r.c0.x, r.c0.y, r.c0.z, r.c0.w, r.c1.x, r.c1.y, r.c1.z, r.c1.w};
#pragma unroll
    for (int i = 0; i < 8; ++i) {
        f[2 * i] = __uint_as_float(w[i] << 16);
        f[2 * i + 1] = __uint_as_float(w[i] & 0xffff0000u);
    }
}
__device__ __forceinline__ Raw pack(const float (&f)[16]) {
    unsigned w[8];
#pragma unroll
    for (int i = 0; i < 8; ++i) w[i] = (unsigned)f2bf(f[2 * i]) | ((unsigned)f2bf(f[2 * i + 1]) << 16);
    Raw r;
    r.c0 = make_uint4(w[0], w[1], w[2], w[3]);
    r.c1 = make_uint4(w[4], w[5], w[6], w[7]);
    return r;
}
__device__ __forceinline__ int col_of(int lane, int j) { return (j < 8 ? 0 : 512) + 8 * lane + (j & 7); }

__device__ __forceinline__ void ld_vec16(const float* __restrict__ v, int lane, float (&f)[16]) {
#pragma unroll
    for (int h = 0; h < 2; ++h) {
        const float4 a = *reinterpret_cast<const float4*>(v + h * 512 + 8 * lane);
        const float4 b = *reinterpret_cast<const float4*>(v + h * 512 + 8 * lane + 4);
        f[8 * h + 0] = a.x; f[8 * h + 1] = a.y; f[8 * h + 2] = a.z; f[8 * h + 3] = a.w;
        f[8 * h + 4] = b.x; f[8 * h + 5] = b.y; f[8 * h + 6] = b.z; f[8 * h + 7] = b.w;
    }
}
}
}
```

egopack_amd/data.py:

```python
from __future__ import annotations

import math
from dataclasses import dataclass
from typing import List, Optional, Sequence

import numpy as np
import torch


class Data:

    def __init__(self, **kw):
        for k, v in kw.items():
            setattr(self, k, v)

    def __contains__(self, key):
        return getattr(self, key, None) is not None

    def materialise(self):
        return self

    def keys(self):
        return [k for k, v in self.materialise().__dict__.items() if v is not None]

# ... 8 lines not shown
                v = [t.to(device, non_blocking=non_blocking) for t in v]
            setattr(out, k, v)
        return out

    def pin_memory(self):
        for k, v in self.materialise().__dict__.items():
            if torch.is_tensor(v) or isinstance(v, CSRGraph):
                setattr(self, k, v.pin_memory())
        return self


class LazyData(Data):

    fills = 0

    def __init__(self, fill):
        self.__dict__["_fill"] = fill

    def materialise(self):
        fill = self.__dict__.pop("_fill", None)
        if fill is not None:
            LazyData.fills += 1
            for k, v in fill().items():
                self.__dict__.setdefault(k, v)
        return self

    def __getattr__(self, name):
        if name.startswith("__") or "_fill" not in self.__dict__:
            raise AttributeError(name)
        self.materialise()
        try:
            return self.__dict__[name]
        except KeyError:
            raise AttributeError(name) from None


HEAVY_DEGREE = 24
HEAVY_IN_LAUNCH_DEGREE = 64


@dataclass
class CSRGraph:
    rowptr: torch.Tensor
    col: torch.Tensor
    t_rowptr: torch.Tensor
    t_col: torch.Tensor
    t_wgt: torch.Tensor
    num_nodes: int
    heavy: Optional[torch.Tensor] = None
    t_heavy: Optional[torch.Tensor] = None
    heavy_mode: int = 0
    t_heavy_mode: int = 0
    band: Optional[torch.Tensor] = None

    def _map(self, f):
        return CSRGraph(*(f(t) for t in (self.rowptr, self.col, self.t_rowptr, self.t_col, self.t_wgt)), self.num_nodes,
                        *(f(t) if t is not None else None for t in (self.heavy, self.t_heavy)), self.heavy_mode, self.t_heavy_mode,
                        f(self.band) if self.band is not None else None)

    def to(self, device, non_blocking: bool = False):
        return self._map(lambda t: t.to(device, non_blocking=non_blocking))

    def pin_memory(self):
        return self._map(lambda t: t.pin_memory())


def build_csr(edge_index: torch.Tensor, num_nodes: int) -> CSRGraph:
    dev = edge_index.device
    src, tgt = edge_index[0].long(), edge_index[1].long()
    deg_in = torch.bincount(tgt, minlength=num_nodes)
    order = torch.argsort(tgt, stable=True)
    rowptr = torch.zeros(num_nodes + 1, dtype=torch.int64, device=dev)
    rowptr[1:] = torch.cumsum(deg_in, 0)
    col = src[order]
    deg_out = torch.bincount(src, minlength=num_nodes)
    t_order = torch.argsort(src, stable=True)
    t_rowptr = torch.zeros(num_nodes + 1, dtype=torch.int64, device=dev)
    t_rowptr[1:] = torch.cumsum(deg_out, 0)
    t_col = tgt[t_order]
    t_wgt = 1.0 / deg_in[t_col].clamp(min=1).to(torch.float32)
    heavy = torch.nonzero(deg_in > HEAVY_DEGREE).flatten().int()
    t_heavy = torch.nonzero(deg_out > HEAVY_DEGREE).flatten().int()
    mode = lambda deg, listed: int(listed.numel() > 0 and int(deg.max()) <= HEAVY_IN_LAUNCH_DEGREE)
    return CSRGraph(rowptr.int(), col.int(), t_rowptr.int(), t_col.int(), t_wgt, int(num_nodes), heavy, t_heavy,
                    mode(deg_in, heavy), mode(deg_out, t_heavy), band_codes(rowptr, col, num_nodes))


def band_codes(rowptr: torch.Tensor, col: torch.Tensor, num_nodes: int) -> torch.Tensor:
    n = int(num_nodes)
    deg = (rowptr[1:] - rowptr[:-1]).long()
    row_of = torch.repeat_interleave(torch.arange(n, device=col.device), deg)
    off = col.long() - row_of
    near = off.abs() <= 1
    bad = torch.zeros(n, dtype=torch.bool, device=col.device)
    bad |= deg > 3
    if col.numel():
        bad.index_put_((row_of[~near],), torch.ones(int((~near).sum()), dtype=torch.bool, device=col.device), accumulate=False)
        same_row = row_of[1:] == row_of[:-1]
        unordered = same_row & (off[1:] <= off[:-1])
        bad.index_put_((row_of[1:][unordered],), torch.ones(int(unordered.sum()), dtype=torch.bool, device=col.device), accumulate=False)
    bits = torch.zeros(n, dtype=torch.int64, device=col.device)
    if col.numel():
        ok = near
        bits.index_add_(0, row_of[ok], (1 << (off[ok] + 1)).long())
    code = torch.where(bad, torch.full_like(bits, 0xFF), bits.clamp(max=7))
    return code.to(torch.uint8)


def radius_band_edges(pos: torch.Tensor, k: int, max_num_neighbors: int = 32) -> torch.Tensor:
    p = pos.reshape(-1).to(torch.int64)
    n = p.numel()
    d = (p.view(-1, 1) - p.view(1, -1)).abs()
    adj = (d.to(torch.float64) <= (k + 0.5)) & ~torch.eye(n, dtype=torch.bool)
    tgt, src = adj.nonzero(as_tuple=True)
    if max_num_neighbors is not None and n > max_num_neighbors:
        deg = torch.bincount(tgt, minlength=n)
        start = torch.cumsum(deg, 0) - deg
        keep = (torch.arange(tgt.numel()) - start[tgt]) < max_num_neighbors
        tgt, src = tgt[keep], src[keep]
    return torch.stack([src, tgt])


def lta_connectivity_edges(pos: torch.Tensor, y: torch.Tensor, r: float) -> torch.Tensor:
    n = pos.shape[0]
    band = radius_band_edges(pos, int(math.floor(r)))
    n_in = int((y[:, 0] == -1).sum())
    n_f = int((y[:, 0] > 0).sum())
    lo = max(math.ceil(n_in - r), 0)
    src = torch.arange(lo, n_in, dtype=torch.long).repeat_interleave(n_f)
    tgt = torch.arange(n_in, n_in + n_f, dtype=torch.long).repeat(min(math.floor(r), n_in))
    ei = torch.cat([torch.stack([src, tgt]), band], dim=-1)
    key = torch.unique(ei[0] * n + ei[1], sorted=True)
    return torch.stack([key // n, key % n])


class RadiusGraph:

    def __init__(self, r: float, loop: bool = False, max_num_neighbors: int = 32, flow: str = "source_to_target"):
# ... 96 lines not shown
    return out


def merge_batches(batches: Sequence[Data]) -> Data:
    if batches and all(b.__dict__.get("_arena") is not None and b.__dict__["_arena"].layout.kind == "task" for b in batches):
        return _merge_arenas(batches)
    poss, eis, seg = [], [], [0]
    off = 0
    for b in batches:
        poss.append(b.pos)
        eis.append(b.edge_index + off)
        off += b.pos.shape[0]
        seg.append(off)
    ei = torch.cat(eis, dim=1)
    xs = [b.x for b in batches]
    base = getattr(batches[0], "x_base", None)
    x = base if (base is not None and all(getattr(b, "x_base", None) is base for b in batches)
                 and base.shape[0] == off) else xs
    out = Data(x=x, pos=torch.cat(poss), edge_index=ei)
    graphs = [getattr(b, "graph", None) for b in batches]
    out.graph = concat_csr(graphs) if all(g is not None for g in graphs) else build_csr(ei, off)
    out.seg_ptr = torch.tensor(seg, dtype=torch.int32)
    out.num_segments = len(batches)
    out.min_seg_rows = min(b - a for a, b in zip(seg, seg[1:]))
    if all(getattr(b, "pos_range", None) is not None for b in batches):
        out.pos_range = (min(b.pos_range[0] for b in batches), max(b.pos_range[1] for b in batches))
    return out


def concat_csr(graphs: Sequence[CSRGraph]) -> CSRGraph:
    def ptr(name):
        parts, eoff = [], 0
        for g in graphs:
            rp = getattr(g, name)
            parts.append(rp[:-1] + eoff)
            eoff += int(rp[-1])
        parts.append(torch.tensor([eoff], dtype=torch.int32, device=parts[0].device))
        return torch.cat(parts).to(torch.int32)

    def ids(name):
        parts, noff = [], 0
        for g in graphs:
            v = getattr(g, name)
            parts.append((v if v is not None else torch.zeros(0, dtype=torch.int32)) + noff)
            noff += g.num_nodes
        return torch.cat(parts).to(torch.int32)

    def mode(listed, name):
        with_rows = [getattr(g, name) for g, l in zip(graphs, listed) if l is not None and l.numel()]
        return int(bool(with_rows) and all(m == 1 for m in with_rows))
    heavy, t_heavy = ids("heavy"), ids("t_heavy")
    band = torch.cat([g.band for g in graphs]) if all(g.band is not None for g in graphs) else None
    rowptr_all, col_all = ptr("rowptr"), ids("col")
    return CSRGraph(rowptr_all, col_all, ptr("t_rowptr"), ids("t_col"), torch.cat([g.t_wgt for g in graphs]),
                    sum(g.num_nodes for g in graphs), heavy, t_heavy, mode([g.heavy for g in graphs], "heavy_mode"),
                    mode([g.t_heavy for g in graphs], "t_heavy_mode"), band)


class PinnedRing:

    def __init__(self, depth: int = 3):
        self.depth, self.slots, self.next = depth, {}, {}

    def get(self, shape, dtype) -> "tuple[torch.Tensor, list]":
        key = (tuple(shape), dtype)
        ring = self.slots.setdefault(key, [])
        i = self.next.get(key, 0)
        if len(ring) < self.depth:
            ring.append([torch.empty(shape, dtype=dtype, pin_memory=True), None])
            i = len(ring) - 1
        self.next[key] = (i + 1) % self.depth
        slot = ring[i]
        if slot[1] is not None:
            slot[1].synchronize()
            slot[1] = None
        return slot[0], slot


_pinned_ring = PinnedRing()
_NUMPY_DTYPES = frozenset((torch.int64, torch.int32, torch.int16, torch.int8, torch.uint8, torch.bool, torch.float32,
                           torch.float64, torch.float16))


EDGE_FIELDS = (".edge_index", ".graph.col", ".graph.t_col", ".graph.t_wgt")
EDGE_BUCKET = 1024


def edge_capacity(e: int) -> int:
    return (int(e) + EDGE_BUCKET - 1) // EDGE_BUCKET * EDGE_BUCKET


class BlobRef:

    def __init__(self, dev, gsig, rebuild):
        self.dev, self.gsig, self.rebuild = dev, gsig, rebuild
        self.names = None


_NP_OF = {torch.int64: "int64", torch.int32: "int32", torch.uint8: "uint8", torch.float32: "float32", torch.float64: "float64",
          torch.int16: "int16", torch.int8: "int8", torch.bool: "bool"}


class ArenaLayout:

    def __init__(self, kind: str, fields, edge_cap: int):
        import numpy as np
        self.kind, self.edge_cap = kind, int(edge_cap)
        self.fields, self.offs, off = [], {}, 0
        for name, shape, dt, edge in fields:
            cap = self.edge_cap if edge else 0
            stored = (*shape[:-1], cap) if cap else tuple(shape)
            nbytes = int(np.prod(stored, dtype=np.int64)) * torch.empty(0, dtype=dt).element_size()
            self.fields.append((name, off, tuple(shape), dt, cap, nbytes))
            self.offs[name] = off
            off += (nbytes + 255) // 256 * 256
        self.total = max(off, 256)
        self.token = hash((kind, tuple((n, o, (*sh[:-1], c) if c else sh, str(dt)) for n, o, sh, dt, c, _ in self.fields)))

    def views(self, buf: torch.Tensor, base: int, E: int, static: bool = False, only=None) -> dict:
        out = {}
        for name, off, shape, dt, cap, nbytes in self.fields:
            if only is not None and name not in only:
                continue
            if not nbytes:
                out[name] = torch.empty((*shape[:-1], E) if cap else shape, dtype=dt, device=buf.device)
            elif cap:
                region = buf[base + off:base + off + nbytes].view(dt).view((*shape[:-1], cap))
                out[name] = region if static else region[..., :E]
            else:
                out[name] = buf[base + off:base + off + nbytes].view(dt).view(shape)
        return out


class Arena:

    def __init__(self, buf, layout: ArenaLayout, E: int, meta: dict):
        self.buf, self.layout, self.E, self.meta = buf, layout, int(E), meta
        self.sig = tuple(sorted(meta.items()))

    def addr(self, name: str) -> int:
        return self.buf.ctypes.data + self.layout.offs[name]


_ARENA_EAGER = ("num_graphs", "pos_range", "live_ap", "num_segments", "min_seg_rows")


def _arena_fields(layout: ArenaLayout, meta: dict, buf: torch.Tensor, base: int, E: int, static: bool = False) -> dict:
    v = layout.views(buf, base, E, static)
    g = CSRGraph(v["graph.rowptr"], v["graph.col"], v["graph.t_rowptr"], v["graph.t_col"], v["graph.t_wgt"], meta["num_nodes"],
                 v["graph.heavy"], v["graph.t_heavy"], meta["heavy_mode"], meta["t_heavy_mode"], v["graph.band"])
    if layout.kind == "merged":
        out = dict(x=None, pos=v["pos"], edge_index=v["edge_index"], graph=g, seg_ptr=v["seg_ptr"],
                   num_segments=meta["num_segments"], min_seg_rows=meta["min_seg_rows"])
        if "pos_range" in meta:
            out["pos_range"] = meta["pos_range"]
        return out
    out = dict(x=None, y=v["y"], pos=v["pos"], edge_index=v["edge_index"], batch=v["batch"], ptr=v["ptr"], num_graphs=meta["num_graphs"])
    if "pos_range" in meta:
        out["pos_range"] = meta["pos_range"]
    out.update(x_idx=v["x_idx"], graph=g, ptr32=v["ptr32"], seg_ptr=v["seg_ptr"])
    if "live_idx" in v:
        out.update(live_idx=v["live_idx"], live_inv=v["live_inv"], live_y=v["live_y"])
        if "live_ap" in meta:
            out["live_ap"] = meta["live_ap"]
    for name in v:
        if name.startswith("attr."):
            out[name[5:]] = v[name]
    return out


def arena_batch(arena: Arena) -> "LazyData":
    host = torch.from_numpy(arena.buf)
    out = LazyData(lambda: _arena_fields(arena.layout, arena.meta, host, 0, arena.E))
    d = out.__dict__
    d["_arena"] = arena
    d["x"] = None
    for k in _ARENA_EAGER:
        if k in arena.meta:
            d[k] = arena.meta[k]
    if arena.layout.kind == "task":
        d["x_idx"] = arena.layout.views(host, 0, arena.E, only=("x_idx",))["x_idx"]
    return out


def _merge_arenas(batches: Sequence["Data"]) -> "Data":
    import ctypes as C
    import numpy as np
    from . import _lib
    ars = [b._arena for b in batches]
    k = len(ars)
    parts = (_lib.HostPart * k)()
    N = E = nh = nth = 0
    for p, a in zip(parts, ars):
        m, lay = a.meta, a.layout
        p.n_nodes, p.E, p.n_heavy, p.n_t_heavy = m["num_nodes"], a.E, m["n_heavy"], m["n_t_heavy"]
        p.edge_stride = lay.edge_cap or a.E
        p.pos_min, p.pos_max = m["pos_range"]
        p.heavy_mode, p.t_heavy_mode = m["heavy_mode"], m["t_heavy_mode"]
        base = a.buf.ctypes.data
        for name, fld in _PART_PTRS:
            setattr(p, fld, base + lay.offs[name])
        N, E, nh, nth = N + p.n_nodes, E + a.E, nh + p.n_heavy, nth + p.n_t_heavy
    key = (k, N, edge_capacity(E), nh, nth)
    lay = _merged_layouts.get(key)
    if lay is None:
        i64, i32 = torch.int64, torch.int32
        lay = _merged_layouts[key] = ArenaLayout("merged", [
            ("pos", (N,), i64, False), ("edge_index", (2, E), i64, True), ("graph.rowptr", (N + 1,), i32, False),
            ("graph.col", (E,), i32, True), ("graph.t_rowptr", (N + 1,), i32, False), ("graph.t_col", (E,), i32, True),
            ("graph.t_wgt", (E,), torch.float32, True), ("graph.heavy", (nh,), i32, False), ("graph.t_heavy", (nth,), i32, False),
            ("graph.band", (N,), torch.uint8, False), ("seg_ptr", (k + 1,), i32, False)], edge_capacity(E))
    buf = np.empty(lay.total, dtype=np.uint8)
    base = buf.ctypes.data
    om = _lib.HostMerged(edge_cap=lay.edge_cap, **{fld: base + lay.offs[name] for name, fld in _MERGED_PTRS})
    rc = int(_lib.load().egk_host_merge_batches(parts, k, C.byref(om)))
    if rc != 0:
        raise ValueError(f"egk_host_merge_batches failed (code {rc})")
    meta = dict(num_nodes=N, n_heavy=nh, n_t_heavy=nth, heavy_mode=int(om.heavy_mode), t_heavy_mode=int(om.t_heavy_mode),
                num_segments=k, min_seg_rows=int(om.min_seg_rows), pos_range=(int(om.pos_min), int(om.pos_max)))
    out = arena_batch(Arena(buf, lay, E, meta))
    xs = [b.__dict__.get("x") for b in batches]
    base_x = batches[0].__dict__.get("x_base")
    out.x = base_x if (base_x is not None and all(b.__dict__.get("x_base") is base_x for b in batches)
                       and base_x.shape[0] == N) else xs
    return out


_merged_layouts = {}
_BATCH_PTRS = (("y", "y"), ("pos", "pos"), ("batch", "batch"), ("ptr", "ptr"), ("ptr32", "ptr32"), ("x_idx", "x_idx"),
               ("edge_index", "edge_index"), ("graph.rowptr", "rowptr"), ("graph.col", "col"), ("graph.t_rowptr", "t_rowptr"),
               ("graph.t_col", "t_col"), ("graph.t_wgt", "t_wgt"), ("graph.band", "band"), ("graph.heavy", "heavy"),
               ("graph.t_heavy", "t_heavy"))
_BATCH_PTRS_LIVE = (*_BATCH_PTRS, ("live_idx", "live_idx"), ("live_inv", "live_inv"), ("live_y", "live_y"))
_PART_PTRS = (("pos", "pos"), ("edge_index", "edge_index"), ("graph.rowptr", "rowptr"), ("graph.col", "col"),
              ("graph.t_rowptr", "t_rowptr"), ("graph.t_col", "t_col"), ("graph.t_wgt", "t_wgt"), ("graph.band", "band"),
              ("graph.heavy", "heavy"), ("graph.t_heavy", "t_heavy"))
_MERGED_PTRS = (*_PART_PTRS, ("seg_ptr", "seg_ptr"))


def _pack_arenas(datas, device, non_blocking: bool, on_gpu: bool) -> List["Data"]:
    ars = [d._arena for d in datas]
    bases, total = [], 0
    for a in ars:
        bases.append(total)
        total += (a.layout.total + 255) // 256 * 256
    size = (total + 65535) // 65536 * 65536
    if on_gpu:
        host, slot = _pinned_ring.get((size,), torch.uint8)
    else:
        host, slot = torch.empty(size, dtype=torch.uint8), None
    hn = host.numpy()
    for a, b in zip(ars, bases):
        hn[b:b + a.layout.total] = a.buf
    if on_gpu:
        dev = host.to(device, non_blocking=non_blocking)
        ev = torch.cuda.Event()
        ev.record(torch.cuda.current_stream())
        slot[1] = ev
    else:
        dev = host.clone()
    specs = [(a.layout, a.meta, b, a.E) for a, b in zip(ars, bases)]

    def rebuild(buf, static: bool = False, lazy: bool = False):
        outs = []
        for lay, meta, b, E in specs:
            if lazy:
                ld = LazyData(lambda lay=lay, meta=meta, b=b, E=E: _arena_fields(lay, meta, buf, b, E, static))
                ld.__dict__["x"] = None
                for k in _ARENA_EAGER:
                    if k in meta:
                        ld.__dict__[k] = meta[k]
                if lay.kind == "task":
                    ld.__dict__["x_idx"] = lay.views(buf, b, E, static, only=("x_idx",))["x_idx"]
                outs.append(ld)
            else:
                outs.append(Data(**_arena_fields(lay, meta, buf, b, E, static)))
        return outs
    outs = rebuild(dev, lazy=True)
# ... 457 lines not shown
            em = max(int(e.max()), 1)
            EI = np.zeros((n, 2, em), dtype=np.int64)
            COL, TCOL, TW = np.zeros((n, em), dtype=np.int64), np.zeros((n, em), dtype=np.int64), np.zeros((n, em), dtype=np.float32)
            RP, TRP, BAND = np.zeros((n, T + 1), dtype=np.int64), np.zeros((n, T + 1), dtype=np.int64), np.zeros((n, T), dtype=np.uint8)
            nh = np.array([g.heavy.numel() for _, g in self.items], dtype=np.int64)
            nth = np.array([g.t_heavy.numel() for _, g in self.items], dtype=np.int64)
            HV, THV = np.zeros((n, max(int(nh.max()), 1)), dtype=np.int64), np.zeros((n, max(int(nth.max()), 1)), dtype=np.int64)
            dmax, tdmax = np.zeros(n, dtype=np.int64), np.zeros(n, dtype=np.int64)
            for i, (ei, g) in enumerate(self.items):
                k = ei.shape[1]
                EI[i, :, :k] = ei
                COL[i, :k], TCOL[i, :k], TW[i, :k] = g.col.numpy(), g.t_col.numpy(), g.t_wgt.numpy()
                RP[i], TRP[i], BAND[i] = g.rowptr.numpy(), g.t_rowptr.numpy(), g.band.numpy()
                HV[i, :nh[i]], THV[i, :nth[i]] = g.heavy.numpy(), g.t_heavy.numpy()
                dmax[i] = int(np.diff(RP[i]).max()) if T else 0
                tdmax[i] = int(np.diff(TRP[i]).max()) if T else 0
            self._tables = dict(e=e, EI=EI, COL=COL, TCOL=TCOL, TW=TW, RP=RP, TRP=TRP, BAND=BAND, nh=nh, nth=nth, HV=HV, THV=THV,
                                dmax=dmax, tdmax=tdmax)
        return self._tables

    def assemble(self, tau):
        import numpy as np
        t, T = self.tables(), self.T
        tau = np.asarray(tau, dtype=np.int64)
        B = tau.shape[0]
        key = tau.tobytes()
        hit = self._assembled.get(key) if hasattr(self, "_assembled") else None
        if hit is not None:
            return hit
        if not hasattr(self, "_assembled"):
            self._assembled = {}
        e = t["e"][tau]
        eoff, noff = np.cumsum(e) - e, np.arange(B, dtype=np.int64) * T
        E = int(e.sum())
        ei, sample_of, pos_in = _ragged(t["EI"], t["e"], tau)
        shift = noff[sample_of]
        ei = (ei.T if ei.ndim == 2 else ei.reshape(2, 0)) + shift[None, :]
        col = t["COL"][tau[sample_of], pos_in] + shift
        t_col = t["TCOL"][tau[sample_of], pos_in] + shift
        t_wgt = t["TW"][tau[sample_of], pos_in]
        rowptr = np.concatenate([(t["RP"][tau][:, :T] + eoff[:, None]).ravel(), [E]])
        t_rowptr = np.concatenate([(t["TRP"][tau][:, :T] + eoff[:, None]).ravel(), [E]])
        band = t["BAND"][tau].ravel()

        def listed(table, counts, dm):
            if not int(counts[tau].sum()):
                return torch.zeros(0, dtype=torch.int32), 0
            v, so, _ = _ragged(table, counts, tau)
            return torch.from_numpy((v + noff[so]).astype(np.int32)), int(int(dm[tau].max()) <= HEAVY_IN_LAUNCH_DEGREE)
        heavy, mode = listed(t["HV"], t["nh"], t["dmax"])
        t_heavy, t_mode = listed(t["THV"], t["nth"], t["tdmax"])
        i32 = lambda a: torch.from_numpy(np.ascontiguousarray(a, dtype=np.int32))
        graph = CSRGraph(i32(rowptr), i32(col), i32(t_rowptr), i32(t_col), torch.from_numpy(np.ascontiguousarray(t_wgt)), B * T,
                         heavy, t_heavy, mode, t_mode, torch.from_numpy(np.ascontiguousarray(band)))
        out = (torch.from_numpy(np.ascontiguousarray(ei)), graph)
        if len(self._assembled) < 64:
            self._assembled[key] = out
        return out


class SyntheticResidentDataset(SyntheticTaskDataset):

    def __init__(self, task: str, length: int, T: int, num_segments: int = 3, features_size: int = 1536,
                 num_class_labels=(115, 478), k: int = 1, seed: int = 1, transform=None, split: str = "train",
                 n_videos: int = 4, frames: int = 600):
        super().__init__(task, length, T, num_segments, features_size, num_class_labels, k, seed, transform)
        import numpy as np
        self.split = split
        rs = np.random.RandomState(seed)
        self.videos = {f"video_{v}": rs.standard_normal((frames, features_size)).astype(np.float32) for v in range(n_videos)}
        self.first_row, off = {}, 0
        for uid, arr in self.videos.items():
            self.first_row[uid] = off
            off += arr.shape[0]
        self.windows = []
        for i in range(length):
            uid = f"video_{int(rs.randint(n_videos))}"
            starts = np.sort(rs.randint(0, frames - 8, size=T))
            lens = rs.randint(0, 40, size=T)
            self.windows.append((uid, starts, starts + lens))
        self.rng = np.random.RandomState(seed + 17)

    def _labels(self, i: int):
        return SyntheticTaskDataset.__getitem__(self, i, with_x=False)

    def _rows(self, i: int):
        import numpy as np
        from .feature_store import window_rows
        uid, starts, ends = self.windows[i]
        n = self.videos[uid].shape[0]
        rows = [window_rows(self.first_row[uid], n, int(a), int(b), self.S, self.split == "train", self.rng)
                for a, b in zip(starts, ends)]
        return np.stack(rows)

    def __getitem__(self, i: int) -> Data:
        d = self._labels(i)
        d.x_idx = torch.from_numpy(self._rows(i))
        return d

    def _tables(self):
        import numpy as np
        tb = getattr(self, "_batch_tables", None)
        if tb is None:
            tmpl = GraphTemplates(self.T)
            ys, poss, tau, scalars = [], [], [], {}
            for i in range(self.length):
                d = self._labels(i)
# ... 50 lines not shown
        from . import _lib
        from .feature_store import _mt_commit, _mt_state
        tb = self._tables()
        nt = self._native_tables()
        if (nt["n_templates"] != len(tb["tmpl"].items) or nt["hil"] != int(HEAVY_IN_LAUNCH_DEGREE)
                or nt["share"] != float(LIVE_ROWS_MAX_SHARE)):
            self._native = None
            nt = self._native_tables()
        idx = np.ascontiguousarray(list(chunk) if not isinstance(chunk, np.ndarray) else chunk, dtype=np.int64)
        B, T, S, heads = int(idx.shape[0]), self.T, self.S, nt["heads"]
        if B == 0:
            return self.batch_numpy(chunk)
        lib, n = _lib.load(), B * T
        sizes = nt["sizes"]
        rc = int(lib.egk_host_batch_sizes(C.byref(nt["desc"]), idx.ctypes.data, B, sizes.ctypes.data))
        if rc != 0:
            raise ValueError(f"batch: sample index out of range (egk_host_batch_sizes: code {rc})")
        E, nh, nth, n_live = (int(v) for v in sizes)
        live_cap = max(64, (n_live + 63) // 64 * 64) if n_live >= 0 else 0
        key = (B, edge_capacity(E), nh, nth, live_cap)
        lay = nt["layouts"].get(key)
        if lay is None:
            i64, i32 = torch.int64, torch.int32
            ys = nt["y_shape"]
            y_shape = (n, *ys[1:]) if (len(ys) >= 1 and ys != (1,)) else (B * int(np.prod(ys, dtype=np.int64)),)
            fields = [("y", y_shape, i64, False), ("pos", (n,), i64, False), ("edge_index", (2, E), i64, True), ("batch", (n,), i64, False),
                      ("ptr", (B + 1,), i64, False), ("x_idx", (n, S), i64, False), ("graph.rowptr", (n + 1,), i32, False),
                      ("graph.col", (E,), i32, True), ("graph.t_rowptr", (n + 1,), i32, False), ("graph.t_col", (E,), i32, True),
                      ("graph.t_wgt", (E,), torch.float32, True), ("graph.heavy", (nh,), i32, False), ("graph.t_heavy", (nth,), i32, False),
                      ("graph.band", (n,), torch.uint8, False), ("ptr32", (B + 1,), i32, False), ("seg_ptr", (2,), i32, False)]
            if live_cap:
                fields += [("live_idx", (live_cap,), i64, False), ("live_inv", (n,), i64, False), ("live_y", (live_cap, heads), i64, False)]
            fields += [(f"attr.{k}", (B,), torch.from_numpy(v[:1]).dtype, False) for k, v in tb["scalars"].items()]
            lay = nt["layouts"][key] = ArenaLayout("task", fields, edge_capacity(E))
        buf = np.empty(lay.total, dtype=np.uint8)
        base, offs = buf.ctypes.data, lay.offs
        ob = _lib.HostBatch(E=E, heavy_cap=nh, t_heavy_cap=nth, live_cap=live_cap, edge_cap=lay.edge_cap,
                            **{fld: base + offs[name] for name, fld in (_BATCH_PTRS_LIVE if live_cap else _BATCH_PTRS)})
        if self.split == "train":
            state, mkey, mpos = _mt_state(self.rng)
            rc = int(lib.egk_host_build_batch(C.byref(nt["desc"]), mkey.ctypes.data, mpos.ctypes.data, idx.ctypes.data, B, C.byref(ob)))
            if rc == 0:
                _mt_commit(self.rng, state, mkey, mpos)
        else:
            rc = int(lib.egk_host_build_batch(C.byref(nt["desc"]), None, None, idx.ctypes.data, B, C.byref(ob)))
        if rc != 0 or int(ob.n_live) != n_live:
            raise ValueError(f"egk_host_build_batch failed (code {rc})")
        seg = buf[offs["seg_ptr"]:offs["seg_ptr"] + 8].view(np.int32)
        seg[0], seg[1] = 0, n
        for k, v in tb["scalars"].items():
            o = offs[f"attr.{k}"]
            buf[o:o + B * v.itemsize].view(v.dtype)[:] = v[idx]
        meta = dict(num_graphs=B, num_nodes=n, n_heavy=nh, n_t_heavy=nth, heavy_mode=int(ob.heavy_mode), t_heavy_mode=int(ob.t_heavy_mode),
                    pos_range=(int(ob.pos_min), int(ob.pos_max)))
        if live_cap and ob.live_ap_step > 0:
            meta["live_ap"] = (int(ob.live_ap_first), int(ob.live_ap_step), live_cap)
        out = arena_batch(Arena(buf, lay, E, meta))
        out.__dict__["_struct_key"] = hash((id(self), B, nt["keep"]["tau"][idx].tobytes())) or 1
        return out

    def batch_numpy(self, chunk) -> Data:
        import numpy as np
        from .feature_store import window_rows_batch
        tb = self._tables()
        idx = np.asarray(list(chunk), dtype=np.int64)
        B, T = idx.shape[0], self.T
        rows = window_rows_batch(np.repeat(tb["first"][idx], T), np.repeat(tb["vlen"][idx], T), tb["starts"][idx].ravel(),
                                 tb["ends"][idx].ravel(), self.S, self.split == "train", self.rng)
        tn = lambda a: torch.from_numpy(np.ascontiguousarray(a))
        y = tb["y"][idx]
        y = y.reshape(-1, *y.shape[2:]) if y.ndim > 1 and y.shape[1:] != (1,) else y.reshape(-1)
        pos = tb["pos"][idx].reshape(-1)
        ei, graph = tb["tmpl"].assemble(tb["tau"][idx])
        n = B * T
        ptr = np.arange(0, n + 1, T, dtype=np.int64)
        out = Data(x=None, y=tn(y), pos=tn(pos), edge_index=ei, batch=tn(np.repeat(np.arange(B, dtype=np.int64), T)), ptr=tn(ptr),
                   num_graphs=B)
        if n:
            out.pos_range = (int(pos.min()), int(pos.max()))
        out.x_idx = torch.from_numpy(rows)
        out.graph = graph
        out.ptr32 = tn(ptr.astype(np.int32))
        out.seg_ptr = tn(np.array([0, n], dtype=np.int32))
        _attach_live_rows(out)
        for key, v in tb["scalars"].items():
            setattr(out, key, tn(v[idx]))
        return out

    def host_item(self, i: int) -> Data:
        import numpy as np
        d = self._labels(i)
        rows = self._rows(i)
        table = np.concatenate(list(self.videos.values()))
        d.x = torch.from_numpy(np.where(rows[..., None] >= 0, table[np.maximum(rows, 0)], 0.0).astype(np.float32))
        return d
```

egopack_amd/ops.py:

```python
from __future__ import annotations

import contextlib
import ctypes as C
import math
from typing import Optional

import torch

from . import _lib, switches

F32, BF16 = 0, 1
X3 = 2

_MODES = {"bf16": (BF16, torch.bfloat16), "bf16_f32act": (BF16, torch.float32), "f32": (F32, torch.float32),
          "bf16x3": (X3, torch.float32)}
_state = {"mode": "bf16", "compute": BF16, "act": torch.bfloat16}


def set_compute(mode: str) -> None:
    comp, act = _MODES[mode]
    _state.update(mode=mode, compute=comp, act=act)


def get_compute() -> str:
# ... 1965 lines not shown
        table = None
        if 0 < n_pos <= 4096:
            fid = _pe_freq_id(freq)
            table = _pe_table(freq, fid, pos_range[0], n_pos, cols) if fid is not None else None
        posc, fr = pos.contiguous(), _f32c(freq)
        taped = _tape_take("pe_add", x)
        if taped is not None:
            return _r16(taped, "y")
        if slabbed and table is None:
            x = _c(x)
            slabbed = False
        tee = _tee_arm(y)
        if table is not None:
            xin, took = _slab_consumer(x) if slabbed else (None, False)
            _ck(lib.egk_pe_add_table(_stream(), xin if took else _p(x), _p(posc), _p(fr), _p(table), int(pos_range[0]), int(n_pos),
                                     _p(y), rows, cols, _dt(x)), "egk_pe_add_table")
            if took:
                _slabs_written(x)
        else:
            _ck(lib.egk_pe_add(_stream(), _p(x), _p(posc), _p(fr), _p(y), rows, cols, _dt(x)), "egk_pe_add")
        _tee_done(y, tee)
        _tape_put("pe_add", y=y)
        return y

    @staticmethod
    def backward(ctx, dy):
        return dy, None, None, None


def pe_add(x, pos, freq, pos_range=None):
    if pos.dtype != torch.int64:
        pos = pos.to(torch.int64)
    return _PEAdd.apply(x, pos, freq, pos_range)


def _csr_gather(x, rowptr, col, wgt, gate, out, heavy=None, heavy_mode=0, band=None):
    lib = _lib.load()
    rows, cols = x.shape
    nh = int(heavy.numel()) if heavy is not None else 0
    ws = workspace(lib.egk_csr_heavy_ws_bytes(nh, cols), x.device) if nh and not heavy_mode else None
    tee = _tee_arm(out) if (wgt is None and gate is None and (nh == 0 or heavy_mode)) else None
    if band is not None and wgt is None and gate is None:
        _ck(lib.egk_csr_gather_banded(_stream(), _p(x), _p(rowptr), _p(col), _p(band), _p(out), rows, cols, _dt(x),
                                      _p(heavy) if nh else None, nh, _p(ws) if ws is not None else None, int(heavy_mode)),
            "egk_csr_gather_banded")
        _tee_done(out, tee)
        return
    _ck(lib.egk_csr_gather(_stream(), _p(x), _p(rowptr), _p(col), _p(wgt), _p(gate), _p(out), rows, cols, _dt(x),
                           _p(heavy) if nh else None, nh, _p(ws) if ws is not None else None, int(heavy_mode)), "egk_csr_gather")
    _tee_done(out, tee)



class _CSRMean(torch.autograd.Function):
    @staticmethod
    def forward(ctx, x, rowptr, col, t_rowptr, t_col, t_wgt, heavy, t_heavy, heavy_mode=0, t_heavy_mode=0, band=None):
        _need_gpu(x, rowptr, col)
        x = _c(x)
        out = torch.empty_like(x)
        _csr_gather(x, rowptr, col, None, None, out, heavy, heavy_mode, band)
        ctx.save_for_backward(t_rowptr, t_col, t_wgt, t_heavy)
        ctx.t_heavy_mode = t_heavy_mode
        return out

    @staticmethod
    def backward(ctx, dout):
        t_rowptr, t_col, t_wgt, t_heavy = ctx.saved_tensors
        dout = _c(dout)
        dx = torch.empty_like(dout)
        _csr_gather(dout, t_rowptr, t_col, t_wgt, None, dx, t_heavy, ctx.t_heavy_mode)
        return dx, None, None, None, None, None, None, None, None, None, None


def csr_mean_aggregate(x, graph):
    return _CSRMean.apply(x, graph.rowptr, graph.col, graph.t_rowptr, graph.t_col, graph.t_wgt,
                          getattr(graph, "heavy", None), getattr(graph, "t_heavy", None), getattr(graph, "heavy_mode", 0),
                          getattr(graph, "t_heavy_mode", 0), getattr(graph, "band", None))


class _SageMean(torch.autograd.Function):

    @staticmethod
    def forward(ctx, h, Wp, bp, Wl, bl, Wr, rowptr, col, t_rowptr, t_col, t_wgt, compute, heavy=None, t_heavy=None,
                heavy_mode=0, t_heavy_mode=0, ln_out=None, ln_in=None, res_src=None, band=None):
        _need_gpu(h, Wp, Wl, Wr)
        lib = _lib.load()
        h = _c(h)
        N, H = h.shape
        dt = h.dtype
        Wp_o, Wl_o, Wr_o = weight_operand(Wp, dt), weight_operand(Wl, dt), weight_operand(Wr, dt)
        xp = torch.empty_like(h)
        agg = torch.empty_like(h)
        p_args, p_kw = (N, H, h, H, Wp_o, H, H, xp, H), dict(bias=_f32c(bp), act=1, compute=compute)
        taped = _tape_take("sage_mean", h)
        Ho = Wl.shape[0]
        if taped is not None:
            xp, agg, out = _r16(taped, "xp"), _r16(taped, "agg"), _r16(taped, "out")
            if tuple(out.shape) != (N, Ho):
                raise RuntimeError("dual_replay: a taped SAGE layer result has another shape")
            if ln_out is not None:
                ln_out["partials"] = None
            ctx.t_heavy_mode = t_heavy_mode
        else:
            gemm(*p_args, **p_kw)
            _csr_gather(xp, rowptr, col, None, None, agg, heavy, heavy_mode, band)
            ctx.t_heavy_mode = t_heavy_mode
            out = torch.empty((N, Ho), dtype=dt, device=h.device)
            c_args = (N, Ho, agg, H, Wl_o, H, H, out, Ho)
            c_kw = dict(A2=h, lda2=H, B2=Wr_o, ldb2=H, K2=H, bias=_f32c(bl), compute=compute)
            if ln_out is not None and _ln_fusion["on"]:
                ln_out["partials"] = _gemm_with_stats(c_args, c_kw, dict(mode=1, seg_ptr=ln_out["seg_ptr"], n_seg=ln_out["n_seg"],
                                                                         min_rows=ln_out["min_rows"]))
            else:
                _gemm_deferrable(c_args, c_kw, slab_ok=ln_out is not None)
            _tape_put("sage_mean", xp=xp, agg=agg, out=out)
        ctx.ln_in, ctx.res_src = ln_in, res_src
        ctx.compute, ctx.params = compute, (Wp, bp, Wl, bl, Wr)
        ctx.save_for_backward(h, xp, agg, Wp_o, Wl_o, Wr_o, t_rowptr, t_col, t_wgt, t_heavy)
        return out

    @staticmethod
    def backward(ctx, d_out):
        lib = _lib.load()
        stamp("bwd_sage", seq=True)
        h, xp, agg, Wp_o, Wl_o, Wr_o, t_rowptr, t_col, t_wgt, t_heavy = ctx.saved_tensors
        Wp, bp, Wl, bl, Wr = ctx.params
        g = _operand_rows(d_out, h.dtype)
        N, H = h.shape
        Ho = g.shape[1]
        dev = g.device

        def slot_or_zeros(p, shape):
            s_ = _grad_slot(p)
            return (s_, None) if s_ is not None else ((z := torch.zeros(shape, dtype=torch.float32, device=dev)), z)

        dWl, rWl = slot_or_zeros(Wl, Wl_o.shape)
        dbl, rbl = slot_or_zeros(bl, (Ho,))
        dWr, rWr = slot_or_zeros(Wr, Wr_o.shape)
        dWp, rWp = slot_or_zeros(Wp, Wp_o.shape)
        dbp, rbp = slot_or_zeros(bp, (H,))
        in_place = rWl is None and rbl is None and rWr is None

        l_args, l_kw = (Ho, H, g, g.stride(0), agg, H, N, dWl, H), dict(transA=True, transB=True, accumulate=True,
                                                                        compute=ctx.compute, dbias=dbl)
        r_args, r_kw = (Ho, H, g, g.stride(0), h, H, N, dWr, H), dict(transA=True, transB=True, accumulate=True, compute=ctx.compute)

        def launch_out_grads():
            gemm(*l_args, **l_kw)
            gemm(*r_args, **r_kw)
        park = (in_place and ctx.compute in (BF16, F32) and not _on_excluded_stream()
                and _wgrad_groupable(Ho, H, g, g.stride(0), agg, H, N, ctx.compute)
                and _wgrad_groupable(Ho, H, g, g.stride(0), h, H, N, ctx.compute))
        if park:
            if not _wgrad_defer(l_args, l_kw, (g, agg)):
                raise RuntimeError("sage_mean_layer: a weight gradient announced as parkable was refused")
            if not _wgrad_defer(r_args, r_kw, (g, h)):
                raise RuntimeError("sage_mean_layer: a weight gradient announced as parkable was refused")
        else:
            _wgrad_launch(in_place, (g, agg, h), launch_out_grads)
        d_agg = torch.empty_like(h)
        d_pre = torch.empty_like(h)
        a_args, a_kw = (N, H, g, g.stride(0), Wl_o, H, Ho, d_agg, H), dict(transB=True, compute=ctx.compute)
        gemm(*a_args, **a_kw)
        _csr_gather(d_agg, t_rowptr, t_col, t_wgt, xp, d_pre, t_heavy, ctx.t_heavy_mode)
        d_h = None
        if ctx.needs_input_grad[0]:
            d_h = torch.empty_like(h)
            h_args = (N, H, g, g.stride(0), Wr_o, H, Ho, d_h, H)
            h_kw = dict(A2=d_pre, lda2=H, B2=Wp_o, ldb2=H, K2=H, transB=True, compute=ctx.compute)
            extra = ctx.res_src.pop("dy", None) if ctx.res_src is not None else None
            if extra is not None:
                if tuple(extra.shape) != tuple(d_h.shape):
                    raise RuntimeError("sage_mean_layer: the handed-over gradient does not have the layer input's shape")
                h_kw.update(residual=_c(extra), ldr=H)
            if ctx.ln_in is not None:
                _ln_bwd_stats_launch(ctx.ln_in, h_args, h_kw, d_h)
            else:
                gemm(*h_args, **h_kw)
        p_args, p_kw = (H, H, d_pre, H, h, H, N, dWp, H), dict(transA=True, transB=True, accumulate=True, compute=ctx.compute,
                                                               dbias=dbp)
        if not (rWp is None and rbp is None and ctx.compute in (BF16, F32) and _wgrad_defer(p_args, p_kw, (d_pre, h))):
            _wgrad_launch(rWp is None and rbp is None, (d_pre, h), lambda: gemm(*p_args, **p_kw))
        if ctx.res_src is not None and _last_wgrad["tail"] is not None:
            flush_wgrad()
        return (d_h, rWp, rbp, rWl, rbl, rWr, None, None, None, None, None, None, None, None, None, None, None, None, None, None)


def sage_mean_layer(h, conv, graph, compute=None, ln_out=None, ln_in=None, res_src=None):
    return _SageMean.apply(h, conv.lin.weight, conv.lin.bias, conv.lin_l.weight, conv.lin_l.bias, conv.lin_r.weight,
                           graph.rowptr, graph.col, graph.t_rowptr, graph.t_col, graph.t_wgt,
                           _compute_for(h) if compute is None else compute, getattr(graph, "heavy", None),
                           getattr(graph, "t_heavy", None), getattr(graph, "heavy_mode", 0), getattr(graph, "t_heavy_mode", 0),
                           ln_out, ln_in, res_src, getattr(graph, "band", None))


class _LiveRows(torch.autograd.Function):

    @staticmethod
    def forward(ctx, x, idx, inv):
        _need_gpu(x)
        x = _c(x)
        idx, inv = idx.contiguous(), inv.contiguous()
        out = torch.empty((idx.numel(), x.shape[1]), dtype=x.dtype, device=x.device)
        _ck(_lib.load().egk_gather_rows(_stream(), _p(x), _dt(x), x.stride(0), x.shape[0], _p(idx), _p(out), _dt(out), idx.numel(),
                                        x.shape[1]), "egk_gather_rows")
        ctx.save_for_backward(inv)
        return out

    @staticmethod
    def backward(ctx, g):
        inv, = ctx.saved_tensors
        g = _c(g)
        out = torch.empty((inv.numel(), g.shape[1]), dtype=g.dtype, device=g.device)
        _ck(_lib.load().egk_gather_rows(_stream(), _p(g), _dt(g), g.stride(0), g.shape[0], _p(inv), _p(out), _dt(out), inv.numel(),
                                        g.shape[1]), "egk_gather_rows")
        return out, None, None


def live_rows(x, idx, inv):
    return _LiveRows.apply(x, idx, inv)


@torch.no_grad()
def expand_rows(v, inv, out=None):
    v2 = _c(v.detach().reshape(-1, 1))
    inv = inv.contiguous()
    if out is None:
        out = torch.empty(inv.numel(), dtype=v2.dtype, device=v2.device)
    _ck(_lib.load().egk_gather_rows(_stream(), _p(v2), _dt(v2), 1, v2.shape[0], _p(inv), _p(out), _dt(out), inv.numel(), 1),
        "egk_gather_rows")
    return out


@torch.no_grad()
def _edges_by_prototype(nn: torch.Tensor, K: int):
    flat = nn.reshape(-1)
    srt, perm = torch.sort(flat, stable=True)
    rowptr = torch.zeros(K + 1, dtype=torch.int32, device=nn.device)
    rowptr[1:] = torch.cumsum(torch.bincount(srt, minlength=K), 0).to(torch.int32)
    return rowptr, perm.to(torch.int32)


class _GatherMax(torch.autograd.Function):
    @staticmethod
    def forward(ctx, f, bank, nn):
        _need_gpu(f, bank, nn)
# ... 1037 lines not shown
```

egopack_amd/switches.py:

```python
from __future__ import annotations

import os
import warnings

REGISTRY = {
    "wgrad_grouping": (True, "H x H weight gradients parked and issued six at a time as one grouped launch"),
    "deferred_forks": (True, "forked launches are issued one launch late so that the dX chain keeps its hardware queue under capture"),
    "oscc_one_pass": (True, "the OSCC head (max pool, 2-logit classifier, cross entropy) as pool + one launch"),
    "graphone_adam": (True, "EgoPack step: Adam over GraphONE's slice beside the backbone's backward"),
    "grad_store": (True, "gradient slots with one writer per step are stored, not cleared and accumulated (every capture)"),
    "precise_search": (True, "bf16 modes: the features behind the nearest-prototype search come from a forward-only 'bf16x3' pass"),
    "one_pass": (True, "ONE backbone pass: the bf16 training graph is built from the precise pass's taped results"),
    "x3_tee": (True, "row kernels of the precise pass also store the bf16 halves of their f32 result (split tee)"),
    "x3_lazy_input": (True, "the bf16 input of the precise pass is not widened in memory"),
    "graphone_grouped": (True, "GraphONE's stages of all auxiliary tasks as one chain of grouped launches"),
    "one_graph_exchange": (False, "N ranks: ONE hipGraph incl. the RCCL collectives (bench.py's probe decides; the attribute also sets it)"),
    "sharded_update": (False, "N ranks: reduce-scatter -> Adam on 1 / world of the buffers -> all-gather instead of all-reduce + full Adam"),
}

DEBUG = {
    "window_cand": "print the candidate statistics of eager window searches",
    "group_shapes": "print the problems of every grouped contraction launch issued outside a capture",
    "stage_profile": "print a cProfile of the staging thread (engine.StagedBatches) when a training loop's epoch ends",
}

KNOBS = {
    "EGK_LIB_PATH": "another build of libegopack_hip.so (A/B of two builds in one tree)",
}

_seen_env = {}


def _names(var: str) -> list:
    raw = os.environ.get(var, "")
    hit = _seen_env.get(var)
    if hit is not None and hit[0] == raw:
        return hit[1]
    out = [item.strip() for item in raw.split(",") if item.strip()]
    _seen_env[var] = (raw, out)
    unknown = [k for k in out if k not in (DEBUG if var == "EGK_DBG" else REGISTRY)]
    if unknown:
        warnings.warn(f"{var}: unknown switch name(s) {unknown} (see egopack_amd/switches.py)")
    return out


def enabled(name: str) -> bool:
    default = REGISTRY[name][0]
    if name in _names("EGK_DISABLE"):
        return False
    if name in _names("EGK_ENABLE"):
        return True
    return default


def override(name: str):
    REGISTRY[name]
    if name in _names("EGK_DISABLE"):
        return False
    if name in _names("EGK_ENABLE"):
        return True
    return None

# ... 19 lines not shown
```

include/egopack_hip.h:

```cpp
#ifndef EGOPACK_HIP_H
#define EGOPACK_HIP_H

#include <stdint.h>

#ifdef __cplusplus
extern "C" {
#endif

typedef void* egk_stream_t;

enum { EGK_OK = 0, EGK_EINVAL = -1, EGK_EUNSUPPORTED = -2 };
enum { EGK_F32 = 0, EGK_BF16 = 1 };
enum { EGK_COMPUTE_F32 = 0, EGK_COMPUTE_BF16 = 1 };
enum { EGK_ACT_NONE = 0, EGK_ACT_RELU = 1 };

int egk_version(void);
const char* egk_last_error(void);

int egk_prof_enable(int on);
int egk_prof_reset(void);
int egk_prof_count(void);
int egk_prof_get(int id, char* name, int name_len, int64_t* launches, double* total_ms,
                 double* alg_flops, double* alg_bytes);

// ... 308 lines not shown
int egk_dropout_fwd(egk_stream_t s, const void* x, void* y, uint8_t* mask, int64_t n, float p, uint64_t seed,
                    uint64_t offset, const uint64_t* dev_offset, int32_t dtype);
int egk_dropout_bwd(egk_stream_t s, const void* dy, const uint8_t* mask, void* dx, int64_t n, float p, int32_t dtype);
int egk_relu_gate(egk_stream_t s, const void* dy, const void* y, void* dx, int64_t n, int32_t dtype);
int egk_axpby(egk_stream_t s, const float* x, const float* y, float* out, int64_t n, float a, float b);
int egk_fill_scaled(egk_stream_t s, const float* scalar, float coef, float* out, int64_t n);
int egk_sum_scale(egk_stream_t s, const float* x, float* out, int64_t n, float scale, int32_t accumulate);

int egk_zero_fill(egk_stream_t s, void* p, int64_t bytes);
int egk_zero_fill_ranges(egk_stream_t s, void* base, const int64_t* begin, const int64_t* bytes, int32_t n_ranges);

int egk_adam_step(egk_stream_t s, float* p, const void* g, int32_t g_dtype, float* m, float* v, int64_t n,
                  const float* hyper, float beta1, float beta2, float eps, float weight_decay, void* bf16_shadow);
int egk_adam_step_bump(egk_stream_t s, float* p, const void* g, int32_t g_dtype, float* m, float* v, int64_t n,
                       const float* hyper, float beta1, float beta2, float eps, float weight_decay, void* bf16_shadow,
                       void* bf16_lo_shadow, int64_t* bump_word, int64_t bump);
int egk_adam_hyper(egk_stream_t s, const float* src, int64_t* t_dev, double beta1, double beta2, float* hyper);
int egk_grad_sumsq_slots(int64_t n);
int egk_grad_sumsq(egk_stream_t s, const void* g, int32_t g_dtype, int64_t n, double* partials, int32_t n_slots);
int egk_grad_norm_finalize(egk_stream_t s, const double* partials, int32_t n_slots, const float* src, float max_norm, float* hyper,
                           int64_t* t_dev, int32_t* gate, double* stats);
int egk_adam_step_gated(egk_stream_t s, float* p, const void* g, int32_t g_dtype, float* m, float* v, int64_t n,
                        const float* hyper, float beta1, float beta2, float eps, float weight_decay, void* bf16_shadow,
                        void* bf16_lo_shadow, int64_t* bump_word, int64_t bump, const int32_t* gate);

int egk_weighted_sums(egk_stream_t s, const float* const* xs, const int64_t* ns, const float* coefs, int32_t count, float* out);
int egk_weighted_sums_acc(egk_stream_t s, const float* const* xs, const int64_t* ns, const float* coefs, int32_t count, float* out,
                          double* acc);
int egk_fill_scaled_multi(egk_stream_t s, const float* scalar, const float* coefs, float* const* outs, const int64_t* ns,
                          int32_t count);
int egk_copy_blocks(egk_stream_t s, const void* const* srcs, const int64_t* nbytes, void* dst, int32_t count);

int egk_gather_rows(egk_stream_t s, const void* table, int32_t table_dtype, int64_t ld, int64_t table_rows,
                    const int64_t* idx, void* out, int32_t out_dtype, int64_t n, int32_t cols);

int egk_gather_lerp_rows(egk_stream_t s, const void* table, int32_t table_dtype, int64_t ld, int64_t table_rows,
                         const int64_t* lo, const int64_t* hi, const double* w, void* out, int32_t out_dtype, int64_t n,
                         int32_t cols);

int egk_label_rank(egk_stream_t s, const float* logits, int64_t ld, const int64_t* labels, int64_t label_stride,
                   int32_t* rank, int32_t rows, int32_t C);
int egk_edit_distance(egk_stream_t s, const int64_t* pred, int64_t p_sn, int64_t p_sz, int64_t p_sk, const int64_t* label,
                      int64_t l_sn, int64_t l_sz, int32_t* out, int32_t N, int32_t Z, int32_t K);

#ifdef __cplusplus
}
#endif

#include "egopack_optim.h"
#include "egopack_optim_groups.h"
#include "egopack_ema.h"
#include "egopack_ce_balanced.h"
#include "egopack_bce_balanced.h"

#endif
```

Measured before the change: 148,700 clip-seqs/s.

## Fuse SAGE backward neighbour gather into the dX GEMM epilogue for tile-local graphs

Adds a GEMM variant whose epilogue stages the bf16-rounded output tile in LDS, loads the tile's transposed CSR edges into LDS, and performs the weighted neighbour gather with the ReLU gate before writing d_pre. This is used only when every graph fits inside one row tile (a local_mask computed from the edge index). The aim is to drop the d_agg intermediate round trip through HBM and the separate gather launch in each SAGE layer's backward. In exchange it needs extra LDS, adds a serial per-row edge loop to the GEMM epilogue, and falls back to the old path when the conditions are not met.

```diff
diff --git a/__graft_entry__.py b/__graft_entry__.py
--- a/__graft_entry__.py
+++ b/__graft_entry__.py
@@ -17,7 +17,7 @@
     handle = _lib.load()
     missing = [s for s in [*_lib.header_symbols(), *_lib.optim_header_symbols(), *_lib.optim_groups_header_symbols(),
                             *_lib.ema_header_symbols(), *_lib.ce_balanced_header_symbols(),
-                            *_lib.bce_balanced_header_symbols()] if not hasattr(handle, s)]
+                            *_lib.bce_balanced_header_symbols(), *_lib.gemm_gather_header_symbols()] if not hasattr(handle, s)]
     if missing:
         raise RuntimeError(f"libegopack_hip.so does not export: {missing}")
     import egopack_amd.engine
diff --git a/egopack_amd/_lib.py b/egopack_amd/_lib.py
--- a/egopack_amd/_lib.py
+++ b/egopack_amd/_lib.py
@@ -16,6 +16,7 @@
 EMA_HEADER = HERE.parent / "include" / "egopack_ema.h"
 CE_BALANCED_HEADER = HERE.parent / "include" / "egopack_ce_balanced.h"
 BCE_BALANCED_HEADER = HERE.parent / "include" / "egopack_bce_balanced.h"
+GEMM_GATHER_HEADER = HERE.parent / "include" / "egopack_gemm_gather.h"
 
 vp, i32, i64, u64, f32 = C.c_void_p, C.c_int32, C.c_int64, C.c_uint64, C.c_float
 
@@ -91,6 +92,13 @@
 class EmaDesc(C.Structure):
     _fields_ = [("ema", vp), ("decay", C.c_double), ("warmup", i32)]
 
+
+class GatherEpi(C.Structure):
+    _fields_ = [("t_rowptr", vp), ("t_col", vp), ("t_wgt", vp), ("gate", vp), ("ldg", i64), ("out", vp), ("ldo", i64),
+                ("local_mask", i32), ("n_heavy", i32)]
+
+
+LOCAL_BITS = {64: 1, 96: 2, 128: 4, 192: 8, 256: 16}
 
 OPT_ADAM, OPT_ADAMW, OPT_SGD = 0, 1, 2
 
@@ -239,6 +247,12 @@
 }
 
 
+GEMM_GATHER_SIGNATURES = {
+    "egk_gemm_gather_tile_rows": (C.c_int, [C.POINTER(GemmDesc)]),
+    "egk_gemm_gather": (C.c_int, [vp, C.POINTER(GemmDesc), C.POINTER(GatherEpi)]),
+}
+
+
 def _declared(header: Path) -> list:
     text = header.read_text()
     text = re.sub(r"/\*.*?\*/", "", text, flags=re.S)
@@ -267,6 +281,10 @@
 
 def bce_balanced_header_symbols() -> list:
     return _declared(BCE_BALANCED_HEADER)
+
+
+def gemm_gather_header_symbols() -> list:
+    return _declared(GEMM_GATHER_HEADER)
 
 
 _lib = None
@@ -282,7 +300,8 @@
             "(or __graft_entry__.build()).  egopack_amd has no CPU / eager fallback.")
     lib = C.CDLL(str(LIB_PATH))
     for name, (res, args) in [*SIGNATURES.items(), *OPTIM_SIGNATURES.items(), *OPTIM_GROUPS_SIGNATURES.items(),
-                              *EMA_SIGNATURES.items(), *CE_BALANCED_SIGNATURES.items(), *BCE_BALANCED_SIGNATURES.items()]:
+                              *EMA_SIGNATURES.items(), *CE_BALANCED_SIGNATURES.items(), *BCE_BALANCED_SIGNATURES.items(),
+                              *GEMM_GATHER_SIGNATURES.items()]:
         fn = getattr(lib, name)
         fn.restype = res
         fn.argtypes = args
diff --git a/egopack_amd/csrc/common.h b/egopack_amd/csrc/common.h
--- a/egopack_amd/csrc/common.h
+++ b/egopack_amd/csrc/common.h
@@ -173,6 +173,10 @@
 __device__ __forceinline__ float bf2f(bf16_t h) { return __uint_as_float((unsigned)h << 16); }
 __device__ __forceinline__ bf16_t f2bf(float f) { return __builtin_bit_cast(bf16_t, (__bf16)f); }
 
+__device__ __forceinline__ void gather_edge_add(float& acc, float w, float v) { acc += w * v; }
+__device__ __forceinline__ float gather_gate(float gate, float acc) { return gate > 0.f ? acc : 0.f; }
+__device__ __forceinline__ unsigned round2_bf16(float lo, float hi) { return (unsigned)f2bf(lo) | ((unsigned)f2bf(hi) << 16); }
+
 __device__ __forceinline__ float4 ld4t(const float* __restrict__ p, int c, int cols, bool vec) {
     if (vec && c + 4 <= cols) return *reinterpret_cast<const float4*>(p + c);
     float4 v;
diff --git a/egopack_amd/csrc/gemm.hip b/egopack_amd/csrc/gemm.hip
--- a/egopack_amd/csrc/gemm.hip
+++ b/egopack_amd/csrc/gemm.hip
@@ -492,6 +492,89 @@
     }
 }
 
+struct GatherEpi {
+    const int* rowptr;
+    const int* col;
+    const float* wgt;
+    const bf16_t* gate;
+    long long ldg;
+    bf16_t* out;
+    long long ldo;
+};
+
+template <int NI_>
+__device__ __forceinline__ void gather_stage_store(float* stage, const f32x4 (&acc)[NI_][4], float alpha, int row_base, int wn, int lr, int lg) {
+#pragma unroll
+    for (int i = 0; i < NI_; ++i) {
+        const int row = row_base + i * 16 + lr;
+#pragma unroll
+        for (int j = 0; j < 4; ++j) {
+            const int slot = (wn * 16 + j * 4 + lg) ^ (row & 15);
+            f32x4 v;
+#pragma unroll
+            for (int t = 0; t < 4; ++t) v[t] = bf16_to_f32(f32_to_bf16(acc[i][j][t] * alpha));
+            *reinterpret_cast<f32x4*>(stage + row * 128 + slot * 4) = v;
+        }
+    }
+}
+
+constexpr int GATHER_CSR_BYTES = 16384, GATHER_CSR_EDGES = (GATHER_CSR_BYTES - 1024) / 8;
+
+template <int ROWS, int NTHR, typename StageStore>
+__device__ __forceinline__ void gather_finish_tile(const GemmArgs& g, const GatherEpi& ge, const float* stage, unsigned char* csr, int m0,
+                                                   int n0, int tid, StageStore stage_store) {
+    constexpr int RPP = NTHR / 16, NPASS = ROWS / RPP;
+    static_assert(ROWS % RPP == 0 && ROWS + 1 <= 256 && ROWS + 1 <= NTHR, "whole passes; the row bounds fit their KiB, one per thread");
+    int* rp = reinterpret_cast<int*>(csr);
+    int* ej = reinterpret_cast<int*>(csr + 1024);
+    float* ew = reinterpret_cast<float*>(csr + 1024 + 4 * GATHER_CSR_EDGES);
+    const int c8 = tid & 15, n = n0 + c8 * 8;
+    const int rows_here = min(ROWS, g.M - m0);
+    const int eb = ge.rowptr[m0], ee = ge.rowptr[m0 + rows_here];
+    int my_rp = 0;
+    if (tid <= rows_here) my_rp = ge.rowptr[m0 + tid];
+    uint4 gq[NPASS];
+#pragma unroll
+    for (int it = 0; it < NPASS; ++it) {
+        const int m = m0 + it * RPP + (tid >> 4);
+        gq[it] = m < g.M ? *reinterpret_cast<const uint4*>(ge.gate + (long long)m * ge.ldg + n) : make_uint4(0, 0, 0, 0);
+    }
+    stage_store();
+    const bool in_lds = ee - eb <= GATHER_CSR_EDGES;
+    if (tid <= rows_here) rp[tid] = my_rp;
+    if (in_lds)
+        for (int e = eb + tid; e < ee; e += NTHR) {
+            ej[e - eb] = ge.col[e] - m0;
+            ew[e - eb] = ge.wgt[e];
+        }
+    __syncthreads();
+#pragma unroll
+    for (int it = 0; it < NPASS; ++it) {
+        const int row = it * RPP + (tid >> 4), m = m0 + row;
+        if (m >= g.M) continue;
+        const int e0 = rp[row], e1 = rp[row + 1];
+        float a[8] = {0.f, 0.f, 0.f, 0.f, 0.f, 0.f, 0.f, 0.f};
+        for (int e = e0; e < e1; ++e) {
+            const int j = in_lds ? ej[e - eb] : ge.col[e] - m0;
+            const float w = in_lds ? ew[e - eb] : ge.wgt[e];
+            if ((unsigned)j >= (unsigned)ROWS) continue;
+            const f32x4 lo = *reinterpret_cast<const f32x4*>(stage + j * 128 + (((2 * c8) ^ (j & 15)) << 2));
+            const f32x4 hi = *reinterpret_cast<const f32x4*>(stage + j * 128 + (((2 * c8 + 1) ^ (j & 15)) << 2));
+#pragma unroll
+            for (int t = 0; t < 4; ++t) {
+                gather_edge_add(a[t], w, lo[t]);
+                gather_edge_add(a[4 + t], w, hi[t]);
+            }
+        }
+        const unsigned gw[4] = {gq[it].x, gq[it].y, gq[it].z, gq[it].w};
+        unsigned pk[4];
+#pragma unroll
+        for (int t = 0; t < 4; ++t)
+            pk[t] = round2_bf16(gather_gate(__uint_as_float(gw[t] << 16), a[2 * t]), gather_gate(__uint_as_float(gw[t] & 0xffff0000u), a[2 * t + 1]));
+        *reinterpret_cast<uint4*>(ge.out + (long long)m * ge.ldo + n) = make_uint4(pk[0], pk[1], pk[2], pk[3]);
+    }
+}
+
 template <bool BF16C, bool TA, bool TB, typename AT, typename BT>
 __global__ __launch_bounds__(NTHREADS) void gemm_kernel(const GemmArgs g) {
     __shared__ __attribute__((aligned(16))) unsigned char lds[2 * BM * ROWB];
@@ -629,8 +712,9 @@
     else return __builtin_amdgcn_mfma_f32_16x16x32_bf16(__builtin_bit_cast(bf16x8, b), __builtin_bit_cast(bf16x8, a), c, 0, 0, 0);
 }
 
-template <int NSTAGE, bool TRA, bool TRB, int KG, int MB, int NI = 4, bool VIRT = false, bool F16 = false, int LW = 0>
-__device__ __forceinline__ void gemm_pipe_body(const GemmArgs& g, const int bid) {
+template <int NSTAGE, bool TRA, bool TRB, int KG, int MB, int NI = 4, bool VIRT = false, bool F16 = false, int LW = 0, bool GATH = false>
+__device__ __forceinline__ void gemm_pipe_body(const GemmArgs& g, const int bid, const GatherEpi* ge = nullptr) {
+    static_assert(!GATH || (!TRA && !VIRT && !F16), "the gather epilogue: row-major A, bf16, single launches");
     static_assert(KG == 1 || MB == 1, "wave groups and the tall tile are alternatives");
     static_assert(NI == 4 || ((NI == 3 || NI == 2) && !TRA && ((MB == 1 && (KG == 1 || NI == 2)) || (MB == 2 && KG == 1 && NI == 3))),
                   "96- / 64-row tiles: row-major A; two wave groups with 64-row tiles only; the tall 8-wave tile with NI = 3");
@@ -884,7 +968,38 @@
             __syncthreads();
         }
     }
-    if constexpr (KG == 1) {
+    if constexpr (GATH) {
+        __syncthreads();
+        if constexpr (KG == 1) {
+            static_assert(NSTAGE * STAGE >= 32 * NI * MB * 512, "the whole f32 tile is staged in the ring");
+            float* stage = reinterpret_cast<float*>(lds);
+            gather_finish_tile<32 * NI * MB, NTHREADS * MB>(g, *ge, stage, lds + NSTAGE * STAGE, m0, n0, tid,
+                                                            [&]() { gather_stage_store<NI>(stage, acc, g.alpha, wm * 16 * NI, wn, lr, lg); });
+        } else {
+            constexpr int HF = NI / 2;
+            static_assert(KG * NSTAGE * STAGE >= 2 * 4 * HF * 4 * 64 * 16 + 32 * NI * 512, "exchange area + staged tile");
+            f32x4* xch = reinterpret_cast<f32x4*>(lds);
+            float* stage = reinterpret_cast<float*>(lds + 2 * 4 * HF * 4 * 64 * 16);
+            f32x4* mine_out = xch + ((grp * 4 + w) * (HF * 4)) * 64 + lane;
+            const f32x4* theirs = xch + (((1 - grp) * 4 + w) * (HF * 4)) * 64 + lane;
+            f32x4 half[HF][4];
+#pragma unroll
+            for (int i = 0; i < HF; ++i)
+#pragma unroll
+                for (int j = 0; j < 4; ++j) mine_out[(i * 4 + j) * 64] = grp == 0 ? acc[HF + i][j] : acc[i][j];
+            __syncthreads();
+#pragma unroll
+            for (int i = 0; i < HF; ++i)
+#pragma unroll
+                for (int j = 0; j < 4; ++j) {
+                    if (grp == 0) half[i][j] = acc[i][j] + theirs[(i * 4 + j) * 64];
+                    else half[i][j] = theirs[(i * 4 + j) * 64] + acc[HF + i][j];
+                }
+            gather_finish_tile<32 * NI, NTHREADS * KG>(g, *ge, stage, lds + KG * NSTAGE * STAGE, m0, n0, tid, [&]() {
+                gather_stage_store<HF>(stage, half, g.alpha, wm * 16 * NI + grp * 16 * HF, wn, lr, lg);
+            });
+        }
+    } else if constexpr (KG == 1) {
         if constexpr (MB == 1) {
             if (epilogue_rows_ok(g)) gemm_epilogue_rows<NI>(g, acc, lds, m0, n0, wm, wn, lr, lg, z, tid, tm * g.tiles_n + tn);
             else gemm_epilogue<NI, 4>(g, acc, m0, n0, wm * 16 * NI, wn * 64, lr, lg, z);
@@ -983,6 +1098,10 @@
 template <int NSTAGE, bool TRA, bool TRB, int KG, int MB, int NI = 4, bool F16 = false, int LW = 0>
 __global__ __launch_bounds__(NTHREADS * KG * MB + 64 * LW) void gemm_pipe_kernel(const GemmArgs g) {
     gemm_pipe_body<NSTAGE, TRA, TRB, KG, MB, NI, false, F16, LW>(g, blockIdx.x);
+}
+template <int NSTAGE, bool TRB, int KG, int MB, int NI = 4, int LW = 0>
+__global__ __launch_bounds__(NTHREADS * KG * MB + 64 * LW) void gemm_pipe_gather_kernel(const GemmArgs g, const GatherEpi ge) {
+    gemm_pipe_body<NSTAGE, false, TRB, KG, MB, NI, false, false, LW, true>(g, blockIdx.x, &ge);
 }
 
 constexpr int MAX_GROUPS = 8;
@@ -1489,7 +1608,21 @@
     (void)hipFuncSetAttribute((const void*)egk::gemm_pipe_kernel<3, false, true, 1, 2, 3, false, 4>, hipFuncAttributeMaxDynamicSharedMemorySize, 3 * 40960);
     (void)hipFuncSetAttribute((const void*)egk::gemm_pipe_kernel<2, false, false, 2, 1, 2>, hipFuncAttributeMaxDynamicSharedMemorySize, 4 * 24576);
     (void)hipFuncSetAttribute((const void*)egk::gemm_pipe_kernel<2, false, true, 2, 1, 2>, hipFuncAttributeMaxDynamicSharedMemorySize, 4 * 24576);
+#define EGK_GATHER_ATTR(TB)                                                                                                                  \
+    (void)hipFuncSetAttribute((const void*)egk::gemm_pipe_gather_kernel<3, TB, 1, 2, 3, 4>, hipFuncAttributeMaxDynamicSharedMemorySize, 3 * 40960 + egk::GATHER_CSR_BYTES); \
+    (void)hipFuncSetAttribute((const void*)egk::gemm_pipe_gather_kernel<3, TB, 1, 2, 3>, hipFuncAttributeMaxDynamicSharedMemorySize, 3 * 40960 + egk::GATHER_CSR_BYTES);    \
+    (void)hipFuncSetAttribute((const void*)egk::gemm_pipe_gather_kernel<2, TB, 1, 1, 2>, hipFuncAttributeMaxDynamicSharedMemorySize, 65536 + egk::GATHER_CSR_BYTES);        \
+    (void)hipFuncSetAttribute((const void*)egk::gemm_pipe_gather_kernel<2, TB, 1, 1, 3>, hipFuncAttributeMaxDynamicSharedMemorySize, 65536 + egk::GATHER_CSR_BYTES);        \
+    (void)hipFuncSetAttribute((const void*)egk::gemm_pipe_gather_kernel<2, TB, 2, 1>, hipFuncAttributeMaxDynamicSharedMemorySize, 131072 + egk::GATHER_CSR_BYTES);          \
+    (void)hipFuncSetAttribute((const void*)egk::gemm_pipe_gather_kernel<2, TB, 1, 1>, hipFuncAttributeMaxDynamicSharedMemorySize, 65536 + egk::GATHER_CSR_BYTES)
+    EGK_GATHER_ATTR(false);
+    EGK_GATHER_ATTR(true);
+#undef EGK_GATHER_ATTR
     g_lds_attr_set = true;
+}
+static inline int local_bit(int tile_rows) {
+    return tile_rows == 64 ? EGK_LOCAL_64 : tile_rows == 96 ? EGK_LOCAL_96 : tile_rows == 128 ? EGK_LOCAL_128
+           : tile_rows == 192 ? EGK_LOCAL_192 : tile_rows == 256 ? EGK_LOCAL_256 : 0;
 }
 extern "C" int egk_gemm_set_pipeline(int32_t on) {
     const int prev = g_use_pipe;
@@ -1578,7 +1711,8 @@
     return 0;
 }
 
-static int gemm_core(egk_stream_t stream, const egk_gemm_desc* d, int* query_blocks);
+static int gemm_core(egk_stream_t stream, const egk_gemm_desc* d, int* query_blocks, const egk_gather_epi* ge = nullptr,
+                     int* query_rows = nullptr);
 
 extern "C" int egk_gemm(egk_stream_t stream, const egk_gemm_desc* d) { return gemm_core(stream, d, nullptr); }
 
@@ -1588,8 +1722,65 @@
     return rc == 0 ? blocks : 0;
 }
 
-static int gemm_core(egk_stream_t stream, const egk_gemm_desc* d, int* query_blocks) {
+static int gather_desc_check(const egk_gemm_desc* d, const char* who) {
+#define EGK_GG(cond, msg)                                        \
+    do {                                                         \
+        if (!(cond)) {                                           \
+            if (who) set_error("%s: %s", who, msg);              \
+            return EGK_EINVAL;                                   \
+        }                                                        \
+    } while (0)
+    EGK_GG(d != nullptr, "null descriptor");
+    EGK_GG(d->a_dtype == EGK_BF16 && d->b_dtype == EGK_BF16 && d->c_dtype == EGK_BF16 && d->compute == EGK_COMPUTE_BF16 && !d->op_f16,
+           "bf16 operands, a bf16 result and bf16 compute only");
+    EGK_GG(d->N == 1024, "N must be 1024");
+    EGK_GG(d->M >= 0 && d->K1 >= 0 && d->K2 >= 0, "negative size");
+    EGK_GG(!d->transA, "row-major A only");
+    EGK_GG(d->splitk <= 1, "no split K");
+    EGK_GG(!d->bias && d->act == 0 && !d->residual && !d->accumulate && !d->dbias && d->st_mode == 0,
+           "no bias, activation, residual, accumulation, bias gradient or statistics");
+    return 0;
+#undef EGK_GG
+}
+
+extern "C" int egk_gemm_gather_tile_rows(const egk_gemm_desc* d) {
+    if (gather_desc_check(d, nullptr) != 0 || d->M == 0) return 0;
+    int rows = 0;
+    const int rc = gemm_core(nullptr, d, nullptr, nullptr, &rows);
+    return rc == 0 ? rows : 0;
+}
+
+extern "C" int egk_gemm_gather(egk_stream_t stream, const egk_gemm_desc* d, const egk_gather_epi* e) {
+    {
+        const int rc = gather_desc_check(d, "egk_gemm_gather");
+        if (rc) return rc;
+    }
+    EGK_REQUIRE(e != nullptr, "egk_gemm_gather: null gather description");
+    EGK_REQUIRE(e->n_heavy == 0, "egk_gemm_gather: rows listed for the split launches (n_heavy = %d) are summed in another order", (int)e->n_heavy);
+    EGK_REQUIRE(e->t_rowptr && e->t_col && e->t_wgt && e->gate && e->out, "egk_gemm_gather: null pointer");
+    EGK_REQUIRE(aligned_to(4, {e->t_rowptr, e->t_col, e->t_wgt}) && aligned_to(16, {e->gate, e->out}) && e->ldg >= d->N &&
+                    e->ldo >= d->N && e->ldg % 8 == 0 && e->ldo % 8 == 0,
+                "egk_gemm_gather: gate and out need 16-byte aligned rows of at least N elements");
+    if (d->M == 0) return 0;
+    int rows = 0;
+    {
+        const int rc = gemm_core(nullptr, d, nullptr, nullptr, &rows);
+        if (rc) return rc;
+    }
+    if (rows == 0) {
+        set_error("egk_gemm_gather: the pipelined kernels do not take this problem (egk_gemm_gather_tile_rows answers 0)");
+        return EGK_EUNSUPPORTED;
+    }
+    if ((e->local_mask & local_bit(rows)) == 0) {
+        set_error("egk_gemm_gather: local_mask 0x%x lacks the bit of the %d-row tiles of this launch", (unsigned)e->local_mask, rows);
+        return EGK_EUNSUPPORTED;
+    }
+    return gemm_core(stream, d, nullptr, e, nullptr);
+}
+
+static int gemm_core(egk_stream_t stream, const egk_gemm_desc* d, int* query_blocks, const egk_gather_epi* ge, int* query_rows) {
     EGK_REQUIRE(d != nullptr, "egk_gemm: null descriptor");
+    if (query_rows) *query_rows = 0;
     EGK_REQUIRE(d->M >= 0 && d->N >= 0 && d->K1 >= 0 && d->K2 >= 0, "egk_gemm: negative size");
     EGK_REQUIRE(d->compute == EGK_COMPUTE_F32 || d->compute == EGK_COMPUTE_BF16, "egk_gemm: bad compute type");
     EGK_REQUIRE(!d->op_f16, "egk_gemm: op_f16 is a grouped-launch feature (egk_gemm_grouped with >= 2 problems)");
@@ -1601,7 +1792,7 @@
     EGK_REQUIRE(a16 == b16, "egk_gemm: A and B must have the same element type in memory");
     EGK_REQUIRE(!(a16 && d->compute == EGK_COMPUTE_F32), "egk_gemm: bf16 operands need EGK_COMPUTE_BF16");
     EGK_REQUIRE(!(d->accumulate && d->c_dtype != EGK_F32), "egk_gemm: accumulate needs an f32 C");
-    EGK_REQUIRE(d->C != nullptr || d->M == 0 || d->N == 0, "egk_gemm: null C");
+    EGK_REQUIRE(d->C != nullptr || d->M == 0 || d->N == 0 || ge || query_rows, "egk_gemm: null C");
     if (d->M == 0 || d->N == 0) return 0;
     hipStream_t s = (hipStream_t)stream;
 
@@ -1614,6 +1805,7 @@
         if (rc) return rc;
     }
     g.C = d->C; g.ldc = d->ldc;
+    if (ge || query_rows) { g.C = nullptr; g.ldc = d->N; }
     g.c_bf16 = d->c_dtype == EGK_BF16;
     g.c_vec = g.c_bf16 ? ((reinterpret_cast<uintptr_t>(g.C) & 7) == 0 && g.ldc % 4 == 0) : (aligned16(g.C) && g.ldc % 4 == 0);
     g.accumulate = d->accumulate; g.act = d->act; g.alpha = d->alpha;
@@ -1665,7 +1857,7 @@
         }
     }
     if (pipe_ok) {
-        ensure_lds_attr();
+        if (!query_rows) ensure_lds_attr();
         dim3 pblock(NTHREADS);
         const int nwg128 = g.tiles_m * g.tiles_n * g.splitk;
         const int nkt_slab = cdiv(K / 64, g.splitk);
@@ -1732,11 +1924,39 @@
             *query_blocks = (d->st_mode && st_ok) ? g.tiles_m * g.tiles_n : 0;
             return 0;
         }
+        const bool gather_variant = variant == 3 || variant == 5 || variant == 8 || variant == 11 || variant == 16;
+        if (query_rows) {
+            *query_rows = gather_variant ? tile_rows : 0;
+            return 0;
+        }
         if (d->st_mode && !st_ok) {
             set_error("egk_gemm: st_mode %d is not available for this launch (ask egk_gemm_stats_blocks first)", d->st_mode);
             return EGK_EUNSUPPORTED;
         }
         dim3 pgrid(g.tiles_m * g.tiles_n * g.splitk);
+        if (ge) {
+            if (!gather_variant || (ge->local_mask & local_bit(tile_rows)) == 0) {
+                set_error("egk_gemm_gather: the graph is not local to the %d-row tiles of this launch (ask egk_gemm_gather_tile_rows first)", tile_rows);
+                return EGK_EUNSUPPORTED;
+            }
+            const GatherEpi e{ge->t_rowptr, ge->t_col, ge->t_wgt, (const bf16_t*)ge->gate, ge->ldg, (bf16_t*)ge->out, ge->ldo};
+            ProfScope prof(variant == 8 ? KID_GEMM_BF16_NN_R96 + layout : variant == 11 ? KID_GEMM_BF16_NN_R64 + layout
+                           : variant == 16 ? KID_GEMM_BF16_NN_R192 + layout : (variant == 5 ? KID_GEMM_BF16_NN_G2 : KID_GEMM_BF16_NN) + layout, s, flops, bytes);
+#define EGK_PIPE_GATHER(TB)                                                                                                       \
+    do {                                                                                                                          \
+        if (variant == 16 && g_r192_loaders && nkt_slab >= 4)                                                                     \
+            hipLaunchKernelGGL((gemm_pipe_gather_kernel<3, TB, 1, 2, 3, 4>), pgrid, dim3(2 * NTHREADS + 256), 3 * 40960 + GATHER_CSR_BYTES, s, g, e); \
+        else if (variant == 16) hipLaunchKernelGGL((gemm_pipe_gather_kernel<3, TB, 1, 2, 3>), pgrid, dim3(2 * NTHREADS), 3 * 40960 + GATHER_CSR_BYTES, s, g, e); \
+        else if (variant == 11) hipLaunchKernelGGL((gemm_pipe_gather_kernel<2, TB, 1, 1, 2>), pgrid, pblock, 2 * 24576 + GATHER_CSR_BYTES, s, g, e); \
+        else if (variant == 8) hipLaunchKernelGGL((gemm_pipe_gather_kernel<2, TB, 1, 1, 3>), pgrid, pblock, 2 * 28672 + GATHER_CSR_BYTES, s, g, e);  \
+        else if (variant == 5) hipLaunchKernelGGL((gemm_pipe_gather_kernel<2, TB, 2, 1>), pgrid, dim3(2 * NTHREADS), 4 * 32768 + GATHER_CSR_BYTES, s, g, e); \
+        else hipLaunchKernelGGL((gemm_pipe_gather_kernel<2, TB, 1, 1>), pgrid, pblock, 2 * 32768 + GATHER_CSR_BYTES, s, g, e);                       \
+    } while (0)
+            if (d->transB) EGK_PIPE_GATHER(true);
+            else EGK_PIPE_GATHER(false);
+#undef EGK_PIPE_GATHER
+            return check_launch("egk_gemm_gather");
+        }
 #define EGK_PIPE(TA, TB)                                                                                                  \
     do {                                                                                                                  \
         if (variant == 16 && g_r192_loaders && nkt_slab >= 4) {                                                           \
@@ -1779,6 +1999,11 @@
                                dim3(256), 0, s, g);
         }
         return check_launch("egk_gemm");
+    }
+    if (query_rows) return 0;
+    if (ge) {
+        set_error("egk_gemm_gather: the pipelined kernels do not take this problem (ask egk_gemm_gather_tile_rows first)");
+        return EGK_EUNSUPPORTED;
     }
     if (pipe32_ok) {
         ensure_lds_attr();
diff --git a/egopack_amd/csrc/graph_ops.hip b/egopack_amd/csrc/graph_ops.hip
--- a/egopack_amd/csrc/graph_ops.hip
+++ b/egopack_amd/csrc/graph_ops.hip
@@ -386,8 +386,8 @@
 #pragma unroll
             for (int u = 0; u < 8; ++u)
                 if (e + u < e1) {
-                    a0 += w[u] * __uint_as_float(v[u].x << 16); a1 += w[u] * __uint_as_float(v[u].x & 0xffff0000u);
-                    a2 += w[u] * __uint_as_float(v[u].y << 16); a3 += w[u] * __uint_as_float(v[u].y & 0xffff0000u);
+                    gather_edge_add(a0, w[u], __uint_as_float(v[u].x << 16)); gather_edge_add(a1, w[u], __uint_as_float(v[u].x & 0xffff0000u));
+                    gather_edge_add(a2, w[u], __uint_as_float(v[u].y << 16)); gather_edge_add(a3, w[u], __uint_as_float(v[u].y & 0xffff0000u));
                 }
         }
         if (!WGT) {
@@ -396,12 +396,12 @@
         }
         if (GATE) {
             const uint2 gq = *reinterpret_cast<const uint2*>(gate + (long long)row * r1k::COLS + c);
-            a0 = __uint_as_float(gq.x << 16) > 0.f ? a0 : 0.f; a1 = __uint_as_float(gq.x & 0xffff0000u) > 0.f ? a1 : 0.f;
-            a2 = __uint_as_float(gq.y << 16) > 0.f ? a2 : 0.f; a3 = __uint_as_float(gq.y & 0xffff0000u) > 0.f ? a3 : 0.f;
+            a0 = gather_gate(__uint_as_float(gq.x << 16), a0); a1 = gather_gate(__uint_as_float(gq.x & 0xffff0000u), a1);
+            a2 = gather_gate(__uint_as_float(gq.y << 16), a2); a3 = gather_gate(__uint_as_float(gq.y & 0xffff0000u), a3);
         }
         uint2 o;
-        o.x = (unsigned)f2bf(a0) | ((unsigned)f2bf(a1) << 16);
-        o.y = (unsigned)f2bf(a2) | ((unsigned)f2bf(a3) << 16);
+        o.x = round2_bf16(a0, a1);
+        o.y = round2_bf16(a2, a3);
         *reinterpret_cast<uint2*>(out + (long long)row * r1k::COLS + c) = o;
         return;
     }
@@ -430,7 +430,7 @@
                     float v[16];
                     r1k::unpack(t[u], v);
 #pragma unroll
-                    for (int j = 0; j < 16; ++j) acc[j] += w[u] * v[j];
+                    for (int j = 0; j < 16; ++j) gather_edge_add(acc[j], w[u], v[j]);
                 }
         }
         if (!WGT) {
@@ -442,7 +442,7 @@
             float gv[16];
             r1k::unpack(gt, gv);
 #pragma unroll
-            for (int j = 0; j < 16; ++j) acc[j] = gv[j] > 0.f ? acc[j] : 0.f;
+            for (int j = 0; j < 16; ++j) acc[j] = gather_gate(gv[j], acc[j]);
         }
         r1k::st_raw(out + (long long)row * r1k::COLS, lane, r1k::pack(acc));
     }
diff --git a/egopack_amd/csrc/rows1024.h b/egopack_amd/csrc/rows1024.h
--- a/egopack_amd/csrc/rows1024.h
+++ b/egopack_amd/csrc/rows1024.h
@@ -31,7 +31,7 @@
 __device__ __forceinline__ Raw pack(const float (&f)[16]) {
     unsigned w[8];
 #pragma unroll
-    for (int i = 0; i < 8; ++i) w[i] = (unsigned)f2bf(f[2 * i]) | ((unsigned)f2bf(f[2 * i + 1]) << 16);
+    for (int i = 0; i < 8; ++i) w[i] = round2_bf16(f[2 * i], f[2 * i + 1]);
     Raw r;
     r.c0 = make_uint4(w[0], w[1], w[2], w[3]);
     r.c1 = make_uint4(w[4], w[5], w[6], w[7]);
diff --git a/egopack_amd/data.py b/egopack_amd/data.py
--- a/egopack_amd/data.py
+++ b/egopack_amd/data.py
@@ -84,17 +84,48 @@
     heavy_mode: int = 0
     t_heavy_mode: int = 0
     band: Optional[torch.Tensor] = None
+    local_mask: int = 0
 
     def _map(self, f):
         return CSRGraph(*(f(t) for t in (self.rowptr, self.col, self.t_rowptr, self.t_col, self.t_wgt)), self.num_nodes,
                         *(f(t) if t is not None else None for t in (self.heavy, self.t_heavy)), self.heavy_mode, self.t_heavy_mode,
-                        f(self.band) if self.band is not None else None)
+                        f(self.band) if self.band is not None else None, self.local_mask)
 
     def to(self, device, non_blocking: bool = False):
         return self._map(lambda t: t.to(device, non_blocking=non_blocking))
 
     def pin_memory(self):
         return self._map(lambda t: t.pin_memory())
+
+
+LOCAL_HEIGHTS = (64, 96, 128, 192, 256)
+
+
+def local_mask(src, tgt) -> int:
+    import numpy as np
+    a = np.asarray(src).reshape(-1)
+    b = np.asarray(tgt).reshape(-1)
+    if a.size == 0:
+        return (1 << len(LOCAL_HEIGHTS)) - 1
+    known = {}
+
+    def local(h):
+        if h not in known:
+            known[h] = bool(np.array_equal(a // h, b // h))
+            if known[h]:
+                for m in LOCAL_HEIGHTS:
+                    if m % h == 0:
+                        known[m] = True
+        return known[h]
+    return sum(1 << k for k, h in enumerate(LOCAL_HEIGHTS) if local(h))
+
+
+def _csr_local_mask(t_rowptr, t_col) -> int:
+    import numpy as np
+    if t_rowptr.device.type != "cpu" or t_col.device.type != "cpu":
+        return 0
+    rp = t_rowptr.numpy()
+    return local_mask(np.repeat(np.arange(rp.shape[0] - 1, dtype=np.int64), np.diff(rp)), t_col.numpy())
 
 
 def build_csr(edge_index: torch.Tensor, num_nodes: int) -> CSRGraph:
@@ -115,7 +146,8 @@
     t_heavy = torch.nonzero(deg_out > HEAVY_DEGREE).flatten().int()
     mode = lambda deg, listed: int(listed.numel() > 0 and int(deg.max()) <= HEAVY_IN_LAUNCH_DEGREE)
     return CSRGraph(rowptr.int(), col.int(), t_rowptr.int(), t_col.int(), t_wgt, int(num_nodes), heavy, t_heavy,
-                    mode(deg_in, heavy), mode(deg_out, t_heavy), band_codes(rowptr, col, num_nodes))
+                    mode(deg_in, heavy), mode(deg_out, t_heavy), band_codes(rowptr, col, num_nodes),
+                    local_mask(edge_index[0].numpy(), edge_index[1].numpy()) if dev.type == "cpu" else 0)
 
 
 def band_codes(rowptr: torch.Tensor, col: torch.Tensor, num_nodes: int) -> torch.Tensor:
@@ -318,9 +350,10 @@
     heavy, t_heavy = ids("heavy"), ids("t_heavy")
     band = torch.cat([g.band for g in graphs]) if all(g.band is not None for g in graphs) else None
     rowptr_all, col_all = ptr("rowptr"), ids("col")
-    return CSRGraph(rowptr_all, col_all, ptr("t_rowptr"), ids("t_col"), torch.cat([g.t_wgt for g in graphs]),
+    t_rowptr_all, t_col_all = ptr("t_rowptr"), ids("t_col")
+    return CSRGraph(rowptr_all, col_all, t_rowptr_all, t_col_all, torch.cat([g.t_wgt for g in graphs]),
                     sum(g.num_nodes for g in graphs), heavy, t_heavy, mode([g.heavy for g in graphs], "heavy_mode"),
-                    mode([g.t_heavy for g in graphs], "t_heavy_mode"), band)
+                    mode([g.t_heavy for g in graphs], "t_heavy_mode"), band, _csr_local_mask(t_rowptr_all, t_col_all))
 
 
 class PinnedRing:
@@ -414,7 +447,8 @@
 def _arena_fields(layout: ArenaLayout, meta: dict, buf: torch.Tensor, base: int, E: int, static: bool = False) -> dict:
     v = layout.views(buf, base, E, static)
     g = CSRGraph(v["graph.rowptr"], v["graph.col"], v["graph.t_rowptr"], v["graph.t_col"], v["graph.t_wgt"], meta["num_nodes"],
-                 v["graph.heavy"], v["graph.t_heavy"], meta["heavy_mode"], meta["t_heavy_mode"], v["graph.band"])
+                 v["graph.heavy"], v["graph.t_heavy"], meta["heavy_mode"], meta["t_heavy_mode"], v["graph.band"],
+                 meta.get("local_mask", 0))
     if layout.kind == "merged":
         out = dict(x=None, pos=v["pos"], edge_index=v["edge_index"], graph=g, seg_ptr=v["seg_ptr"],
                    num_segments=meta["num_segments"], min_seg_rows=meta["min_seg_rows"])
@@ -483,13 +517,21 @@
     if rc != 0:
         raise ValueError(f"egk_host_merge_batches failed (code {rc})")
     meta = dict(num_nodes=N, n_heavy=nh, n_t_heavy=nth, heavy_mode=int(om.heavy_mode), t_heavy_mode=int(om.t_heavy_mode),
-                num_segments=k, min_seg_rows=int(om.min_seg_rows), pos_range=(int(om.pos_min), int(om.pos_max)))
+                num_segments=k, min_seg_rows=int(om.min_seg_rows), pos_range=(int(om.pos_min), int(om.pos_max)),
+                local_mask=_arena_local_mask(buf, lay, E))
     out = arena_batch(Arena(buf, lay, E, meta))
     xs = [b.__dict__.get("x") for b in batches]
     base_x = batches[0].__dict__.get("x_base")
     out.x = base_x if (base_x is not None and all(b.__dict__.get("x_base") is base_x for b in batches)
                        and base_x.shape[0] == N) else xs
     return out
+
+
+def _arena_local_mask(buf, lay: ArenaLayout, E: int) -> int:
+    import numpy as np
+    cap = lay.edge_cap or E
+    ei = buf[lay.offs["edge_index"]:lay.offs["edge_index"] + 2 * cap * 8].view(np.int64).reshape(2, cap)
+    return local_mask(ei[0, :E], ei[1, :E])
 
 
 _merged_layouts = {}
@@ -1053,7 +1095,7 @@
         t_heavy, t_mode = listed(t["THV"], t["nth"], t["tdmax"])
         i32 = lambda a: torch.from_numpy(np.ascontiguousarray(a, dtype=np.int32))
         graph = CSRGraph(i32(rowptr), i32(col), i32(t_rowptr), i32(t_col), torch.from_numpy(np.ascontiguousarray(t_wgt)), B * T,
-                         heavy, t_heavy, mode, t_mode, torch.from_numpy(np.ascontiguousarray(band)))
+                         heavy, t_heavy, mode, t_mode, torch.from_numpy(np.ascontiguousarray(band)), local_mask(ei[0], ei[1]))
         out = (torch.from_numpy(np.ascontiguousarray(ei)), graph)
         if len(self._assembled) < 64:
             self._assembled[key] = out
@@ -1210,7 +1252,7 @@
             o = offs[f"attr.{k}"]
             buf[o:o + B * v.itemsize].view(v.dtype)[:] = v[idx]
         meta = dict(num_graphs=B, num_nodes=n, n_heavy=nh, n_t_heavy=nth, heavy_mode=int(ob.heavy_mode), t_heavy_mode=int(ob.t_heavy_mode),
-                    pos_range=(int(ob.pos_min), int(ob.pos_max)))
+                    pos_range=(int(ob.pos_min), int(ob.pos_max)), local_mask=_arena_local_mask(buf, lay, E))
         if live_cap and ob.live_ap_step > 0:
             meta["live_ap"] = (int(ob.live_ap_first), int(ob.live_ap_step), live_cap)
         out = arena_batch(Arena(buf, lay, E, meta))
diff --git a/egopack_amd/ops.py b/egopack_amd/ops.py
--- a/egopack_amd/ops.py
+++ b/egopack_amd/ops.py
@@ -2041,6 +2041,36 @@
 
 
 
+gemm_gather_launches = {"n": 0}
+
+
+def _gemm_gather(a_args, a_kw, t_rowptr, t_col, t_wgt, gate, out, local_mask, heavy=None, heavy_mode=0) -> bool:
+    if not (local_mask and switches.enabled("gather_in_dx_epilogue")):
+        return False
+    M, N, A1 = a_args[0], a_args[1], a_args[2]
+    nh = int(heavy.numel()) if heavy is not None else 0
+    if (a_kw.get("compute") != BF16 or A1.dtype != torch.bfloat16 or gate.dtype != torch.bfloat16 or out.dtype != torch.bfloat16
+            or N != 1024 or M == 0 or (nh and not heavy_mode)):
+        return False
+    lib = _lib.load()
+    d = _gemm_desc(*a_args[:7], out, N, **a_kw)
+    d.C = None
+    if lib.egk_gemm_splitk(M, N, _desc_k(d), d.compute) != 1:
+        _x3_release()
+        return False
+    rows = lib.egk_gemm_gather_tile_rows(C.byref(d))
+    if not rows or not (int(local_mask) & _lib.LOCAL_BITS[rows]):
+        _x3_release()
+        return False
+    e = _lib.GatherEpi(_p(t_rowptr), _p(t_col), _p(t_wgt), _p(gate), gate.stride(0), _p(out), out.stride(0), int(local_mask), 0)
+    try:
+        _ck(lib.egk_gemm_gather(_stream(), C.byref(d), C.byref(e)), "egk_gemm_gather")
+    finally:
+        _x3_release()
+    gemm_gather_launches["n"] += 1
+    return True
+
+
 class _CSRMean(torch.autograd.Function):
     @staticmethod
     def forward(ctx, x, rowptr, col, t_rowptr, t_col, t_wgt, heavy, t_heavy, heavy_mode=0, t_heavy_mode=0, band=None):
@@ -2071,7 +2101,7 @@
 
     @staticmethod
     def forward(ctx, h, Wp, bp, Wl, bl, Wr, rowptr, col, t_rowptr, t_col, t_wgt, compute, heavy=None, t_heavy=None,
-                heavy_mode=0, t_heavy_mode=0, ln_out=None, ln_in=None, res_src=None, band=None):
+                heavy_mode=0, t_heavy_mode=0, ln_out=None, ln_in=None, res_src=None, band=None, local_mask=0):
         _need_gpu(h, Wp, Wl, Wr)
         lib = _lib.load()
         h = _c(h)
@@ -2103,7 +2133,7 @@
             else:
                 _gemm_deferrable(c_args, c_kw, slab_ok=ln_out is not None)
             _tape_put("sage_mean", xp=xp, agg=agg, out=out)
-        ctx.ln_in, ctx.res_src = ln_in, res_src
+        ctx.ln_in, ctx.res_src, ctx.local_mask = ln_in, res_src, int(local_mask or 0)
         ctx.compute, ctx.params = compute, (Wp, bp, Wl, bl, Wr)
         ctx.save_for_backward(h, xp, agg, Wp_o, Wl_o, Wr_o, t_rowptr, t_col, t_wgt, t_heavy)
         return out
@@ -2147,11 +2177,13 @@
                 raise RuntimeError("sage_mean_layer: a weight gradient announced as parkable was refused")
         else:
             _wgrad_launch(in_place, (g, agg, h), launch_out_grads)
-        d_agg = torch.empty_like(h)
         d_pre = torch.empty_like(h)
-        a_args, a_kw = (N, H, g, g.stride(0), Wl_o, H, Ho, d_agg, H), dict(transB=True, compute=ctx.compute)
-        gemm(*a_args, **a_kw)
-        _csr_gather(d_agg, t_rowptr, t_col, t_wgt, xp, d_pre, t_heavy, ctx.t_heavy_mode)
+        a_kw = dict(transB=True, compute=ctx.compute)
+        if not _gemm_gather((N, H, g, g.stride(0), Wl_o, H, Ho), a_kw, t_rowptr, t_col, t_wgt, xp, d_pre, ctx.local_mask,
+                            t_heavy, ctx.t_heavy_mode):
+            d_agg = torch.empty_like(h)
+            gemm(N, H, g, g.stride(0), Wl_o, H, Ho, d_agg, H, **a_kw)
+            _csr_gather(d_agg, t_rowptr, t_col, t_wgt, xp, d_pre, t_heavy, ctx.t_heavy_mode)
         d_h = None
         if ctx.needs_input_grad[0]:
             d_h = torch.empty_like(h)
@@ -2172,7 +2204,8 @@
             _wgrad_launch(rWp is None and rbp is None, (d_pre, h), lambda: gemm(*p_args, **p_kw))
         if ctx.res_src is not None and _last_wgrad["tail"] is not None:
             flush_wgrad()
-        return (d_h, rWp, rbp, rWl, rbl, rWr, None, None, None, None, None, None, None, None, None, None, None, None, None, None)
+        return (d_h, rWp, rbp, rWl, rbl, rWr, None, None, None, None, None, None, None, None, None, None, None, None, None, None,
+                None)
 
 
 def sage_mean_layer(h, conv, graph, compute=None, ln_out=None, ln_in=None, res_src=None):
@@ -2180,7 +2213,7 @@
                            graph.rowptr, graph.col, graph.t_rowptr, graph.t_col, graph.t_wgt,
                            _compute_for(h) if compute is None else compute, getattr(graph, "heavy", None),
                            getattr(graph, "t_heavy", None), getattr(graph, "heavy_mode", 0), getattr(graph, "t_heavy_mode", 0),
-                           ln_out, ln_in, res_src, getattr(graph, "band", None))
+                           ln_out, ln_in, res_src, getattr(graph, "band", None), getattr(graph, "local_mask", 0))
 
 
 class _LiveRows(torch.autograd.Function):
diff --git a/egopack_amd/switches.py b/egopack_amd/switches.py
--- a/egopack_amd/switches.py
+++ b/egopack_amd/switches.py
@@ -8,6 +8,7 @@
     "deferred_forks": (True, "forked launches are issued one launch late so that the dX chain keeps its hardware queue under capture"),
     "oscc_one_pass": (True, "the OSCC head (max pool, 2-logit classifier, cross entropy) as pool + one launch"),
     "graphone_adam": (True, "EgoPack step: Adam over GraphONE's slice beside the backbone's backward"),
+    "gather_in_dx_epilogue": (True, "SAGE backward: the transposed neighbour gather inside the epilogue of the contraction that feeds it (tile-local graphs)"),
     "grad_store": (True, "gradient slots with one writer per step are stored, not cleared and accumulated (every capture)"),
     "precise_search": (True, "bf16 modes: the features behind the nearest-prototype search come from a forward-only 'bf16x3' pass"),
     "one_pass": (True, "ONE backbone pass: the bf16 training graph is built from the precise pass's taped results"),
diff --git a/include/egopack_gemm_gather.h b/include/egopack_gemm_gather.h
--- /dev/null
+++ b/include/egopack_gemm_gather.h
@@ -0,0 +1,33 @@
+#ifndef EGOPACK_GEMM_GATHER_H
+#define EGOPACK_GEMM_GATHER_H
+
+#ifdef __cplusplus
+extern "C" {
+#endif
+
+#define EGK_LOCAL_64 1
+#define EGK_LOCAL_96 2
+#define EGK_LOCAL_128 4
+#define EGK_LOCAL_192 8
+#define EGK_LOCAL_256 16
+
+typedef struct egk_gather_epi {
+    const int32_t* t_rowptr;
+    const int32_t* t_col;
+    const float* t_wgt;
+    const void* gate;
+    int64_t ldg;
+    void* out;
+    int64_t ldo;
+    int32_t local_mask;
+    int32_t n_heavy;
+} egk_gather_epi;
+
+int egk_gemm_gather_tile_rows(const egk_gemm_desc* d);
+
+int egk_gemm_gather(egk_stream_t s, const egk_gemm_desc* d, const egk_gather_epi* e);
+
+#ifdef __cplusplus
+}
+#endif
+#endif
diff --git a/include/egopack_hip.h b/include/egopack_hip.h
--- a/include/egopack_hip.h
+++ b/include/egopack_hip.h
@@ -384,5 +384,6 @@
 #include "egopack_ema.h"
 #include "egopack_ce_balanced.h"
 #include "egopack_bce_balanced.h"
+#include "egopack_gemm_gather.h"
 
 #endif
```

Result: slower. 142,200 clip-seqs/s (-4.4%).
